# artiom-matvei/RLAO

Measured on NVIDIA B200. Metric: closed-loop AO env-steps/sec (batched envs), higher is better.
Workload: dtype f32

## Files before the change

### include/aoenv.h

```cpp
#ifndef AOENV_H_
#define AOENV_H_

#include <stdint.h>

#ifdef __cplusplus
extern "C" {
#endif

#define AOENV_MAX_LAYERS 8
#define AOENV_ABI_VERSION 1

int aoenv_abi_version(void);
const char* aoenv_last_error(void);
uint64_t aoenv_launch_count(void);
int aoenv_set_pdl(int enabled);


int aoenv_atm_gather(const float* win, int B, int M, int pitch, int64_t env_stride, int sx, int sy,
                     const int32_t* inner_rc, int nI, int nO, const float* xi,
                     uint64_t seed, uint64_t stream_id, float* zx, int ldz, void* zx_planes, int parts, void* stream);

int aoenv_atm_ring(float* win, int B, int M, int pitch, int64_t env_stride, int64_t win_offset, int nO, const float* X,
                   int ldx, uint64_t* ext, int32_t* flag, int force_rescan, void* stream);

int aoenv_atm_gather_multi(const void* const* wins, const int32_t* sx, const int32_t* sy, const uint64_t* seeds,
                           const uint64_t* stream_ids, int G, int B, int M, int pitch, int64_t env_stride,
                           const int32_t* inner_rc, int nI, int nO, const float* xi, float* zx, int ldz,
                           void* zx_planes, int parts, void* stream);
int aoenv_atm_ring_multi(void* const* wins, const int64_t* win_offsets, void* const* exts, int G, int B, int M,
                         int pitch, int64_t env_stride, int nO, const float* X, int ldx, int32_t* flag,
                         int force_rescan, void* stream);

int aoenv_atm_gather_envs(const void* const* wins, const uint64_t* seeds, const uint64_t* stream_ids, int G,
                          const int32_t* env_idx, int k, int M, int pitch, int64_t env_stride, const int32_t* inner_rc,
                          int nI, int nO, float* zx, int ldz, void* zx_planes, int parts, void* stream);
int aoenv_atm_ring_envs(void* const* wins, const int64_t* win_offsets, void* const* exts, int G, const int32_t* env_idx,
                        int k, int B, int M, int pitch, int64_t env_stride, int nO, const float* X, int ldx, int32_t* flag,
                        void* stream);

int aoenv_atm_compact(const float* src_win, float* dst_win, int B, int M, int pitch, int64_t env_stride, uint64_t* ext,
                      int64_t pos_delta, void* stream);

int aoenv_vk_screens(uint64_t seed, uint32_t screen0, int S, int N, const float* amp, const float* inject, const void* wa_planes,
                     const void* wb_planes, int Kp, int parts, const float* sh_ex, const float* sh_ey, const float* h_amp,
                     const float* h_mx, const float* h_my, void* work_planes, float* work_a, int lda, float* work_b, int ldb,
                     float* dst, int pitch, int64_t env_stride, void* stream);

int aoenv_vk_screens_envs(uint64_t seed, uint32_t screen0, const int32_t* env_idx, int S, int N, const float* amp,
                          const void* wa_planes, const void* wb_planes, int Kp, int parts, const float* sh_ex,
                          const float* sh_ey, const float* h_amp, const float* h_mx, const float* h_my, void* work_planes,
                          float* work_a, int lda, float* work_b, int ldb, float* dst, int pitch, int64_t env_stride,
                          void* stream);

int aoenv_atm_phase(const float* const* h_canvas, const uint64_t* const* h_ext, const int32_t* h_org, int nLayer, int B,
                    int R, int M, int Mc, int pitch, int fp_off, const int32_t* h_row_off, const int32_t* h_col_off,
                    const float* h_wrow, const float* h_wcol, const float* h_weight, float opd_scale, float* opd_out,
                    void* stream);
int aoenv_atm_phase_envs(const float* const* h_canvas, const uint64_t* const* h_ext, const int32_t* h_org, int nLayer,
                         int B, int R, int M, int Mc, int pitch, int fp_off, const int32_t* h_row_off,
                         const int32_t* h_col_off, const float* h_wrow, const float* h_wcol, const float* h_weight,
                         float opd_scale, const int32_t* env_idx, int k, float* opd_out, void* stream);

typedef struct {
  double ratio[2];
  double buff[2];
  double vX, vY;
  uint64_t events;
  uint64_t philox_seed;
  int32_t not_done_once;
  int32_t cur;
  int32_t org[2];
} aoenv_layer_state_t;

typedef struct {
  int32_t nLayer, B, R, M, Mc, pitch, S, nI, nO, ldz, ldx, group_max, parts, fp_off, warp_kernel, use_tc;
  int64_t env_stride;
  uint64_t env_offset;
  double sampling_time, ps_loop;
  float opd_scale, reserved;
  float weight[AOENV_MAX_LAYERS];
  void* maps[AOENV_MAX_LAYERS][2];
  void* ext[AOENV_MAX_LAYERS];
  const void* inner_rc;
  void* zx;
  void* zx_planes;
  void* X;
  void* flag;
  const void* w_f32;
  aoenv_layer_state_t layer[AOENV_MAX_LAYERS];
} aoenv_atm_state_t;

int aoenv_atm_update(aoenv_atm_state_t* state, const void* w_planes, float* opd_out, void* stream);

#define AOENV_SKINNY_MAX_ROWS 8
int aoenv_gemm_tn(const float* X, int ldx, const float* W, int ldw, float* D, int ldd,
                  int M, int N, int K, float alpha, void* stream);

int aoenv_split_bf16(const float* src, int lds, int rows, int K, int parts, void* dst, int ldk, void* stream);
int aoenv_gemm_tn_tc(const void* Xs, const void* Ws, int ldk, int parts, float* D, int ldd, int MX, int NW, int K,
                     float alpha, void* stream);

int aoenv_dm_surface_separable(const float* coefs, int ldc, const int32_t* act_pos, int nA, int nAct, const float* gx,
                               const float* gy, const int32_t* band_x, const int32_t* band_y, const float* wx,
                               const int32_t* j0x, const float* wyp, const int32_t* i0y, int W, int B, int R, float* opd,
                               void* stream);

typedef struct {
  int32_t photon_noise;
  int32_t sensor_emccd;
  int32_t has_fwc;
  int32_t bits;
  float qe;
  float dark_electrons;
  float fwc;
  float gain;
  float readout_noise;
  uint32_t reserved;
  uint64_t seed;
  uint64_t frame_counter;
} aoenv_detector_t;

int aoenv_detector_integrate(float* frame, int B, int rows, int cols, const aoenv_detector_t* det, void* stream);

int aoenv_shwfs_camera(float* frame, const uint8_t* valid, int B, int nS, int n, const aoenv_detector_t* det, int shared_max,
                       int32_t* envmax, void* stream);

int aoenv_set_wfs6_variant(int variant);

int aoenv_shwfs_frame(const float* opd_a, const float* opd_b, const float* pupil, const float* amp,
                      const uint8_t* valid, int B, int nS, int n, float phase_scale,
                      const aoenv_detector_t* det, int shared_max,
                      float* frame, int32_t* envmax, double* stats, void* stream);

int aoenv_shwfs_slopes(const float* frame, const int32_t* envmax, int shared_max, const int32_t* valid_idx,
                       int nV, const float* ref_xy, float inv_units, float threshold_cog, int B, int nS, int n,
                       float* slopes, int lds, void* slope_planes, int parts, void* stream);

typedef struct {
  const float* rows;
  const float* wlr;
  const int32_t* ilr;
  int32_t nActP;
  int32_t WL;
  int32_t t_rows;
  int32_t reserved;
} aoenv_dm_sep_t;

int aoenv_shwfs_fused(const float* opd_a, const float* opd_b, const aoenv_dm_sep_t* dm, const uint8_t* pupil8, float amp0,
                      const int32_t* h_row_start, const int32_t* order, const int32_t* nlit, const int32_t* slot_of, int B,
                      int nS, int n, int cluster, int groups, float phase_scale, const float* ref_xy, int nV, float inv_units,
                      float threshold_cog, float* frame, float* slopes, int lds, void* slope_planes, int parts,
                      int32_t* envmax, double* stats, void* stream);
int aoenv_shwfs_frame_dm(const float* opd_a, const float* opd_b, const aoenv_dm_sep_t* dm, const int32_t* order,
                         const float* pupil, const float* amp, const uint8_t* valid, int B, int nS, int n, float phase_scale,
                         const aoenv_detector_t* det, int shared_max, float* frame, int32_t* envmax, double* stats,
                         void* stream);
int aoenv_shwfs_fused_smem(int nS, int n, int rows_max, int groups, int t_rows, int WL);
int aoenv_dm_rows(const float* coefs, int ldc, const int32_t* act_pos, int nA, int nAct, int nActP, const float* wx,
                  const int32_t* j0x, int W, int B, int R, float* rows, void* stream);

typedef struct {
  int32_t B, nS, n, nV, lds, nA, nAct, nAct2, ldc, ldr, W, rec_parts, use_tc, geometric;
  float phase_scale, inv_units, threshold_cog, leak;
  double n_pupil;
  const void *pupil, *amp, *valid, *order, *valid_idx, *ref_xy;
  void *frame, *envmax, *stats, *slopes, *slope_planes;
  aoenv_dm_sep_t dm;
  const void *rec_planes, *rec_f32;
  void* rec;
  const void* act_idx;
  void* dm_prev;
  const void *act_pos, *wx, *j0x;
} aoenv_sh_step_t;

int aoenv_sh_step(const aoenv_sh_step_t* c, int parts, const float* opd_a, const float* dm_rows_cur, const aoenv_detector_t* det,
                  const float* action, float* coefs_next, float* dm_rows_next, float* obs, float* reward, float* strehl,
                  float* total, float* residual, void* stream);

int aoenv_shwfs_measure_f64(const float* opd, const float* pupil, const float* amp, const uint8_t* valid,
                            const int32_t* valid_idx, int nV, const double* ref_xy, double inv_units, double threshold_cog,
                            int F, int nS, int n, double phase_scale, int shared_max, double* frame, uint64_t* envmax,
                            double* slopes, int lds, void* stream);

int aoenv_shwfs_geometric(const float* opd_a, const float* opd_b, const aoenv_dm_sep_t* dm, const float* pupil,
                          const float* flux, const int32_t* valid_idx, int nV, int B, int nS, int n, float phase_scale,
                          float inv_units, float* slopes, int lds, void* slope_planes, int parts, double* stats, void* stream);

int aoenv_shwfs_geometric_f64(const float* opd, const float* flux, const int32_t* valid_idx, int nV, int F, int nS, int n,
                              double phase_scale, double inv_units, double* slopes, int lds, void* stream);

int aoenv_pyramid_supported(int N);
int aoenv_pyramid_frames(const float* opd_a, const float* opd_b, const float* pupil, const float* amp, const float* lin,
                         const float* mod, const float* mask_s, int B, int R, int N, int nTheta, int bin, float phase_scale,
                         float* work_x1, float* work_yt, float* intensity, float* frame, void* stream);


int aoenv_command_update(const float* action, const int32_t* act_idx, int B, int nA, int nAct2, float leak,
                         float* coefs, float* dm_prev, int ldc, void* stream);

int aoenv_observe(const float* rec, int ldr, const int32_t* act_idx, int B, int nA, int nAct2,
                  const double* stats, double n_pupil, float phase_scale,
                  float* obs, float* reward, float* strehl, float* total, float* residual, void* stream);

int aoenv_normal_fill(uint64_t seed, uint64_t counter, int rows, int cols, int ld, float sigma, float* out, void* planes,
                      int parts, void* stream);
int aoenv_vec_to_img(const float* vec, int ldv, const int32_t* act_idx, int B, int nA, int nAct2, float scale, float* img,
                     void* stream);

int aoenv_psf_peak(const float* opd_a, const float* opd_b, const float* pupil, const float* amp,
                   const void* w1_planes, const float* g2, int B, int R, int N, int os, int win, float phase_scale,
                   void* field_planes, int ldk, float* scratch, float* psf_win, float* psf_max, void* stream);

int aoenv_psf_image(const float* opd_a, const float* opd_b, const float* pupil, const float* amp, const void* w_planes, int B,
                    int R, int N, int os, int win, float phase_scale, void* field_planes, int ldk, float* work_t, void* planes_u,
                    float* work_f, float* psf, float* psf_max, void* stream);

#ifdef __cplusplus
}
#endif
#endif
```

### rlao_b200/OOPAOEnv/OOPAOEnvRazor.py

```python
import contextlib
import ctypes
import importlib
import math
import os
import types

import numpy as np
import torch

from .. import _lib, gemm
from ..Atmosphere import Atmosphere
from ..DeformableMirror import DeformableMirror, DMSurfaceRef
from ..MisRegistration import MisRegistration
from ..ShackHartmann import ShackHartmann
from ..Source import Source
from ..Telescope import Telescope
from ..Zernike import Zernike
from ..calibration.CalibrationVault import CalibrationVault
from ..calibration.InteractionMatrix import InteractionMatrix
from ..tools import linalg


_NVTX = os.environ.get("AOENV_NVTX", "0") not in ("", "0")

# ... 121 lines not shown
        else:
            M2C = torch.eye(self.dm.nValidAct, dtype=torch.float64, device=self.device)
        calib_zonal = InteractionMatrix(ngs=self.source, atm=self.atm, tel=self.tel, dm=self.dm, wfs=self.wfs,
                                        M2C=torch.eye(self.dm.nValidAct, dtype=torch.float64, device=self.device),
                                        stroke=1e-9, nMeasurements=param.get("nMeasurements", 25), noise="off")
        self.calib_zonal = calib_zonal
        calib = CalibrationVault(calib_zonal.D @ M2C)
        self.tel.resetOPD()
        self.dm.coefs = 0
        self._dm_prev = torch.zeros((self.n_envs, self.dm._Kp), dtype=torch.float32, device=self.device)
        self._coefs_buf = torch.zeros((2, self.n_envs, self.dm._Kp), dtype=torch.float32, device=self.device)
        self._coefs_slot = 0
        self.source * self.tel * self.dm * self.wfs
        self.tel + self.atm
        self.calib_CL = calib
        self.M2C_CL = M2C
        nLoop = param.get("nLoop", None)
        self.SR = []
        self._nLoop = nLoop
        self.total = torch.zeros((nLoop, self.n_envs), dtype=torch.float32, device=self.device) if nLoop else None
        self.residual = torch.zeros((nLoop, self.n_envs), dtype=torch.float32, device=self.device) if nLoop else None
        cam.photonNoise = param.get("cam_photonNoise", True)
        cam.readoutNoise = param.get("cam_readoutNoise", 14 if wfs_type == "shackhartmann" else 0)
        self.set_reconstructor(M2C @ calib.M)
        self.F = M2C @ linalg.pinv(M2C)
        nA_, Kp_ = self.dm.nValidAct, self.dm._Kp
        self._F32 = torch.zeros((nA_, Kp_), dtype=torch.float32, device=self.device)
        self._F32[:, :nA_] = self.F.to(torch.float32)
        self._F_op = gemm.Operator(self._F32, parts=2)
        self.dm.free_float64()
        B, nA = self.n_envs, self.dm.nValidAct
        self._act_idx = torch.as_tensor((self.xvalid * nAct + self.yvalid).astype(np.int32), device=self.device)
        self._rec = torch.zeros((B, (nA + 3) // 4 * 4), dtype=torch.float32, device=self.device)
        self._obs = torch.zeros((B, nAct, nAct), dtype=torch.float32, device=self.device)
        self._reward = torch.zeros((B,), dtype=torch.float32, device=self.device)
        self._strehl = torch.zeros((B,), dtype=torch.float32, device=self.device)
        self._total_now = torch.zeros((B,), dtype=torch.float32, device=self.device)
        self._residual_now = torch.zeros((B,), dtype=torch.float32, device=self.device)
        self._phase_scale = 2 * math.pi / self.source.wavelength
        self._noise_seed = (seed * 7919 + 5) & 0xFFFFFFFFFFFFFFFF
        self._noise_calls = 0
        self._noise_z = torch.zeros((B, self.dm._Kp), dtype=torch.float32, device=self.device)
        self._noise_planes = torch.zeros((2, B, self.dm._Kp), dtype=torch.bfloat16, device=self.device)
        self._noise_vec = torch.zeros((B, (nA + 3) // 4 * 4), dtype=torch.float32, device=self.device)

    def set_reconstructor(self, R):
        self.reconstructor = torch.as_tensor(R, dtype=torch.float64, device=self.device)
        nA, nSig = self.reconstructor.shape
        self._Rm = torch.zeros((nA, self.wfs._lds), dtype=torch.float32, device=self.device)
        self._Rm[:, :nSig] = self.reconstructor.to(torch.float32)
        self._Rm_op = gemm.Operator(self._Rm, parts=2)

    @property
    def dm_prev(self):
        d = self._dm_prev[:, :self.dm.nValidAct]
        return d[0] if self.n_envs == 1 else d

    @dm_prev.setter
    def dm_prev(self, val):
        t = torch.as_tensor(val, dtype=torch.float32, device=self.device)
        self._dm_prev.zero_()
        self._dm_prev[:, :self.dm.nValidAct] = t

    def _sq(self, t):
        return t[0] if self.n_envs == 1 else t

    def _observe(self, with_stats):
        lib, st, B, nA = _lib.load(), _lib.stream_ptr(self.device), self.n_envs, self.dm.nValidAct
        sig = self.wfs._signal
        gemm.gemm_tn(sig, self._Rm_op, self._rec, B, nA,
                     x_planes=self.wfs._signal_planes if gemm.uses_tensor_cores(B) else None)
        _lib.check(lib.aoenv_observe(_lib.ptr(self._rec), self._rec.stride(0), _lib.ptr(self._act_idx), B, nA,
                                     self.nActuator ** 2, _lib.ptr(self.wfs._stats) if with_stats else None,
                                     float(self.tel.pixelArea), self._phase_scale, _lib.ptr(self._obs), _lib.ptr(self._reward),
                                     _lib.ptr(self._strehl), _lib.ptr(self._total_now), _lib.ptr(self._residual_now), st),
                   "observe")

    def _action_tensor(self, action):
        a = torch.as_tensor(action, dtype=torch.float32, device=self.device)
        nAct = self.nActuator
        if a.ndim == 2:
            a = a.unsqueeze(0).expand(self.n_envs, -1, -1)
        return a.reshape(self.n_envs, nAct * nAct).contiguous()

    def reset_soft(self):
        self.action_buffer = []
        self._observe(False)
        return self._sq(self._obs).clone()

    def reset(self):
        raise NotImplementedError("reset() rebuilds the whole simulation in the reference (set_params without arguments, "
                                  "OOPAOEnvRazor.py:66-71, which raises there too); use set_params(...) then reset_soft()")

    def reset_envs(self, env_ids, seed):
        atm, dm = self.atm, self.dm
        atm._check_partial_reset()
        idx = atm.env_index(env_ids)
        if idx.numel() == 0:
            return idx
        if dm._coefs_matrix is not None or dm._multi is not None:
            raise NotImplementedError("reset_envs needs per-environment commands (the mirror holds a calibration command matrix)")
        atm._reset_listed(idx, seed)
        rows = idx.long()
        slot = dm._slot
        self._dm_prev[rows] = 0
        for c in {id(t): t for t in (dm._coefs, dm._coefs_of[slot]) if t is not None}.values():
            c[rows] = 0
        if dm._rows is not None and dm._rows_valid[slot]:
            dm._rows[slot][rows] = 0
        if dm._valid[slot]:
            dm._opd[slot][rows] = 0
        return idx

    def reset_soft_wfs(self):
        self.action_buffer = []
        return self.wfs.cam.frame.clone()

    def _native_cfg(self):
        wfs, dm, tel = self.wfs, self.dm, self.tel
        if (not self.native_step or _NVTX or self.psf_reward is not None or type(wfs) is not ShackHartmann or wfs.use_fused
                or not wfs.inline_dm or not dm.lazy_surface or self.atm.user_defined_opd or dm._multi is not None
                or dm._coefs_matrix is not None):
            return None
        src = tel.src
        if wfs._flux_version != getattr(src, "_flux_version", 0) or wfs.current_nPhoton != src.nPhoton:
            return None
        key = (wfs._flux_version, wfs.is_geometric, id(wfs._amp), id(wfs._ref_xy), wfs.slopes_units, wfs.threshold_cog, float(self.leak),
               id(self._Rm_op), id(dm._sep), src.wavelength, id(self._coefs_buf))
        if self._native_key == key:
            return self._native
        self._native_key, self._native = key, None
        tables = dm.fused_tables()
        win = wfs._dm_windows(tables) if tables is not None else None
        if win is None or 2 * math.pi / src.wavelength != self._phase_scale:
            return None
        tc = gemm.uses_tensor_cores(self.n_envs)
        dm._rows_of(dm._slot)
        c = _lib.ShStepStruct()
        c.B, c.nS, c.n, c.nV, c.lds = self.n_envs, wfs.nSubap, wfs.n_pix_subap, wfs.nValidSubaperture, wfs._signal.stride(0)
        c.nA, c.nAct, c.nAct2 = dm.nValidAct, dm.nAct, self.nActuator ** 2
        c.ldc, c.ldr, c.W, c.rec_parts, c.use_tc = self._coefs_buf.stride(1), self._rec.stride(0), tables["W"], self._Rm_op.parts, int(tc)
        c.geometric = int(wfs.is_geometric)
        c.phase_scale, c.inv_units, c.threshold_cog, c.leak = self._phase_scale, 1.0 / wfs.slopes_units, wfs.threshold_cog, self.leak
        c.n_pupil = float(tel.pixelArea)
        keep = [tel._pupil_f, wfs._amp, wfs._valid_u8, wfs._lit_first, wfs._valid_idx, wfs._ref_xy, wfs._frame, wfs._envmax,
                wfs._stats, wfs._signal, wfs._signal_planes, win, self._Rm, self._Rm_op, self._rec, self._act_idx, self._dm_prev,
                tables]
        c.pupil, c.amp, c.valid, c.order = tel._pupil_f.data_ptr(), wfs._amp.data_ptr(), wfs._valid_u8.data_ptr(), wfs._lit_first.data_ptr()
        c.valid_idx, c.ref_xy, c.envmax = wfs._valid_idx.data_ptr(), wfs._ref_xy.data_ptr(), wfs._envmax.data_ptr()
        if wfs.is_geometric:
            c.amp, c.frame = wfs._flux.data_ptr(), None
            keep.append(wfs._flux)
        else:
            c.frame = wfs._frame.data_ptr()
        c.stats, c.slopes, c.slope_planes = wfs._stats.data_ptr(), wfs._signal.data_ptr(), wfs._signal_planes.data_ptr()
        c.dm.wlr, c.dm.ilr, c.dm.nActP, c.dm.WL = win[2].data_ptr(), win[1].data_ptr(), dm._rows.shape[2], win[0]
        c.rec_planes = self._Rm_op.planes().data_ptr() if tc else None
        c.rec_f32, c.rec, c.act_idx, c.dm_prev = self._Rm.data_ptr(), self._rec.data_ptr(), self._act_idx.data_ptr(), self._dm_prev.data_ptr()
        c.act_pos, c.wx, c.j0x = tables["act_pos"].data_ptr(), tables["wx"].data_ptr(), tables["j0x"].data_ptr()
        self._native = (c, keep)
        return self._native

    def _step_native(self, i, action, native, action_ready=None, after_observe=None):
        c = native[0]
        dm, wfs, atm, B, dev = self.dm, self.wfs, self.atm, self.n_envs, self.device
        slot = dm._slot
        atm.update()
        self.tel._set_lazy(atm._opd, DMSurfaceRef(dm, slot))
        det = None if wfs.is_geometric else wfs.cam.as_struct(self.env_offset)
        nAct = self.nActuator
        obs = torch.empty((B, nAct, nAct), dtype=torch.float32, device=dev)
        reward = torch.empty((B,), dtype=torch.float32, device=dev)
        strehl = torch.empty((B,), dtype=torch.float32, device=dev)
        coefs = self._coefs_buf[self._coefs_slot]
        args = [atm._opd.data_ptr(), dm._rows[slot].data_ptr(), ctypes.byref(det) if det is not None else None, None,
                coefs.data_ptr(), dm._rows[slot ^ 1].data_ptr(), obs.data_ptr(), reward.data_ptr(), strehl.data_ptr(),
                self._total_now.data_ptr(), self._residual_now.data_ptr(), _lib.stream_ptr(dev)]
        step, cref = _lib.load().aoenv_sh_step, ctypes.byref(c)
        if atm.can_prefetch() or after_observe is not None or action_ready is not None:
            early = atm.sm_partition is not None or (self.prefetch_early and after_observe is None and action_ready is None)
            if early:
                atm.prefetch()
            _lib.check(step(cref, 1, *args), "sh_step")
            if not early:
                atm.prefetch()
            _lib.check(step(cref, 2, *args), "sh_step")
            if after_observe is not None:
                after_observe(self._sq(obs), self._sq(reward), self._sq(strehl))
            if action_ready is not None:
                torch.cuda.current_stream(dev).wait_event(action_ready)
            args[3] = self._action_tensor(action).data_ptr()
            _lib.check(step(cref, 4, *args), "sh_step")
        else:
            act = self._action_tensor(action)
            args[3] = act.data_ptr()
            _lib.check(step(cref, 7, *args), "sh_step")
        self._coefs_slot ^= 1
        dm._coefs, dm._multi, dm._coefs_matrix, dm._slot = coefs, None, None, slot ^ 1
        dm._coefs_of[slot ^ 1], dm._rows_valid[slot ^ 1], dm._valid[slot ^ 1] = coefs, True, False
        if not wfs.is_geometric:
            wfs.cam.frame = wfs._frame[0] if B == 1 else wfs._frame
        wfs._signal_is_multi = False
        self._obs, self._reward, self._strehl = obs, reward, strehl
        if self.total is not None and i is not None and 0 <= i < self._nLoop:
            self.total[i] = self._total_now
            self.residual[i] = self._residual_now
        s = self._sq(strehl)
        self.SR.append(s)
        self.wfsSignal = wfs.signal
        return self._sq(obs), self._sq(reward), s, False, {"strehl": s}

    def step(self, i, action):
        native = self._native_cfg()
        if native is not None and self.dm._rows_valid[self.dm._slot]:
            return self._step_native(i, action, native)
        obs, reward, strehl, done, info = self._measure_frame(i)
        self._apply_command(action)
        strehl = strehl.clone()
        self.SR[-1] = strehl
        return obs.clone(), reward.clone(), strehl, done, {"strehl": strehl}

    def _step_views(self, i, action, action_ready=None, after_observe=None):
        native = self._native_cfg()
        if native is not None and self.dm._rows_valid[self.dm._slot]:
            return self._step_native(i, action, native, action_ready, after_observe)
        out = self._measure_frame(i, after_observe)
        self._apply_command(action, action_ready)
        return out

    def _measure_frame(self, i, after_observe=None, atmosphere_done=False):
        if not atmosphere_done:
            with _range("aoenv.atmosphere"):
                self.atm.update()
        else:
            self.atm._join_prefetch(consume=True)
        dm_surface = self.dm.surface_ref()
        self.tel._set_lazy(self.atm._opd, dm_surface)
        with _range("aoenv.wfs"):
            self.wfs._measure_terms(self.atm._opd, dm_surface, self.env_offset)
        if not atmosphere_done:
            with _range("aoenv.atmosphere_next"):
                self.atm.prefetch()
        with _range("aoenv.reconstruct"):
            self._observe(True)
        if self.total is not None and i is not None and 0 <= i < self._nLoop:
            self.total[i] = self._total_now
            self.residual[i] = self._residual_now
        strehl = self._sq(self._strehl)
        if self.psf_reward is not None:
            strehl = self.psf_strehl(*self.psf_reward)
        if after_observe is not None:
            after_observe(self._sq(self._obs), self._sq(self._reward), strehl)
        self.SR.append(strehl if self.psf_reward is not None else strehl.clone())
        self.wfsSignal = self.wfs.signal
        return self._sq(self._obs), self._sq(self._reward), strehl, False, {"strehl": strehl}

    def _apply_command(self, action, action_ready=None):
        lib, st, B = _lib.load(), _lib.stream_ptr(self.device), self.n_envs
        if action_ready is not None:
            torch.cuda.current_stream(self.device).wait_event(action_ready)
        action = self._action_tensor(action)
        coefs = self._coefs_buf[self._coefs_slot]
        self._coefs_slot ^= 1
        with _range("aoenv.command"):
            _lib.check(lib.aoenv_command_update(_lib.ptr(action), _lib.ptr(self._act_idx), B, self.dm.nValidAct,
                                                self.nActuator ** 2, ctypes.c_float(self.leak), _lib.ptr(coefs), _lib.ptr(self._dm_prev),
                                                coefs.stride(0), st), "command_update")
            self.dm._set_coefs_batch(coefs)

    def state_dict(self):
        atm = self.atm
        nxt = None
        if atm._prefetched:
            atm._wait_prefetch()
            nxt = atm._opd_next.detach().cpu().clone()
        layers = []
        for i, ly in enumerate(atm._layers):
            layers.append(dict(map=ly.mapShift.detach().cpu().clone(), buff=ly.buff.copy(), ratio=ly.ratio.copy(),
                               notDoneOnce=ly.notDoneOnce, events=ly.events, philox_seed=getattr(ly, "philox_seed", 0),
                               ext=None))
        return dict(version=1, n_envs=self.n_envs, rng=atm.rng, layers=layers, atm_opd=atm._opd.detach().cpu().clone(),
                    atm_opd_next=nxt,
                    coefs=self.dm._coefs.detach().cpu().clone(), dm_prev=self._dm_prev.detach().cpu().clone(),
                    cam_frame_counter=self.wfs.cam.frame_counter, noise_calls=self._noise_calls,
                    SR=[s.detach().cpu().clone() for s in self.SR],
                    total=None if self.total is None else self.total.detach().cpu().clone(),
                    residual=None if self.residual is None else self.residual.detach().cpu().clone())

    def load_state_dict(self, st):
        if st.get("version") != 1 or st["n_envs"] != self.n_envs or st["rng"] != self.atm.rng:
            raise ValueError("state_dict of another environment (n_envs / rng / version differ)")
        if self.atm.rng != "philox":
            raise NotImplementedError("host MT19937 streams (rng='reference') are not checkpointed; use rng='philox'")
        atm, dev = self.atm, self.device
        atm._join_prefetch(consume=False)
        for i, (ly, s_) in enumerate(zip(atm._layers, st["layers"])):
            atm._cur[i] = 0
            atm._org[i] = atm._fresh_origin(i)
            oy, ox = atm._org[i]
            m = s_["map"].to(dev)
            atm._maps[i, 0, :, oy:oy + atm._M, ox:ox + atm._M] = m if m.ndim == 3 else m.unsqueeze(0)
            ly.buff, ly.ratio, ly.notDoneOnce = s_["buff"].copy(), s_["ratio"].copy(), s_["notDoneOnce"]
            ly.events, ly.philox_seed = s_["events"], s_["philox_seed"]
            atm._rescan_extrema(i)
        atm._opd.copy_(st["atm_opd"].to(dev))
        if st.get("atm_opd_next") is not None:
            if atm._opd_next is None:
# ... 145 lines not shown
```

### rlao_b200/ShackHartmann.py

```python
import ctypes as C
import math
import os

import numpy as np
import torch

from . import _lib, gemm
from .DeformableMirror import DMSurfaceRef
from .Detector import Detector

_SUPPORTED_N = (4, 6, 8)


class ShackHartmann:
    def __init__(self, nSubap, telescope, lightRatio, threshold_cog=0.01, is_geometric=False, binning_factor=1,
                 padding_extension_factor=1, threshold_convolution=0.05, shannon_sampling=False, unit_P2V=False):
        self.tag = "shackHartmann"
        self.telescope = telescope
        if telescope.src is None:
            raise AttributeError("The telescope was not coupled to any source object! Make sure to couple it with an src object using src*tel")
        if binning_factor != 1 or padding_extension_factor > 2:
            raise NotImplementedError("binning_factor != 1 / extended field of view are out of scope")
        if getattr(telescope.src, "type", "NGS") == "LGS":
            raise NotImplementedError("LGS spot elongation is out of scope")
        self.device = telescope.device
        self.n_envs = telescope.n_envs
        self._is_geometric = bool(is_geometric)
        self.nSubap = int(nSubap)
        self._lightRatio = lightRatio
        self.binning_factor = 1
        self.zero_padding = 2
        self.padding_extension_factor = padding_extension_factor
        self.threshold_convolution = threshold_convolution
        self.threshold_cog = threshold_cog
        self.shannon_sampling = shannon_sampling
        self.unit_P2V = unit_P2V
        R = telescope.resolution
        if R % self.nSubap != 0:
            raise ValueError("telescope.resolution must be a multiple of nSubap")
        self.n_pix_subap = R // self.nSubap
        if self.n_pix_subap not in _SUPPORTED_N:
            raise NotImplementedError(f"{self.n_pix_subap} pixels per subaperture: compiled sizes are {_SUPPORTED_N}")
        self.n_pix_subap_init = self.n_pix_subap
        self.n_pix_lenslet_init = self.n_pix_subap * self.zero_padding
        self.n_pix_lenslet = self.n_pix_lenslet_init
        self.is_extended = False
        self.is_LGS = False
        self.cam = Detector(round(self.nSubap * self.n_pix_subap))
        self.cam.photonNoise = 0
        self.cam.readoutNoise = 0
        src = telescope.src
        self.fov_lenslet_arcsec = (self.n_pix_subap * 206265 * self.binning_factor / self.padding_extension_factor
                                   * src.wavelength / (telescope.D / self.nSubap)) / (1 + self.shannon_sampling)
        self.fov_pixel_arcsec = self.fov_lenslet_arcsec / self.n_pix_subap
        self.fov_pixel_binned_arcsec = self.fov_lenslet_arcsec / self.n_pix_subap_init
        self.get_camera_frame_multi = False
        self.env_offset = 0
        self.use_fused = os.environ.get("AOENV_WFS", "kernels") == "fused" and not self._is_geometric
        self.keep_frame = False
        self._fused_plans = {}
        self.inline_dm = os.environ.get("AOENV_WFS_INLINE_DM", "1") != "0"
        self._dm_window_cache = {}
        self._last_inputs = None
        ii, jj = np.meshgrid(np.arange(self.nSubap), np.arange(self.nSubap), indexing="ij")
        self.index_x, self.index_y = ii.reshape(-1), jj.reshape(-1)
        self.initialize_flux()
        self._select_valid()
        B = self.n_envs
        self._frame = None if self._is_geometric else torch.zeros((B, R, R), dtype=torch.float32, device=self.device)
        self._envmax = torch.zeros((B,), dtype=torch.int32, device=self.device)
        self._stats = torch.zeros((B, 4), dtype=torch.float64, device=self.device)
        self._signal = torch.zeros((B, self._lds), dtype=torch.float32, device=self.device)
        self._signal_planes = torch.zeros((2, B, self._lds), dtype=torch.bfloat16, device=self.device)
        self._signal_is_multi = False
        self.initialize_wfs()

    def initialize_flux(self, input_flux_map=None):
        src, nS, n = self.telescope.src, self.nSubap, self.n_pix_subap
        flux = np.asarray(src.fluxMap if input_flux_map is None else input_flux_map.T, dtype=np.float64)
        self.photon_per_subaperture = flux.reshape(nS, n, nS, n).sum(axis=(1, 3)).reshape(-1)
        self.photon_per_subaperture_2D = self.photon_per_subaperture.reshape(nS, nS)
        self._amp = torch.as_tensor(np.sqrt(flux), dtype=torch.float32, device=self.device).contiguous()
        if self._is_geometric:
            self._flux = torch.as_tensor(flux, dtype=torch.float32, device=self.device).contiguous()
        self.current_nPhoton = src.nPhoton
        self._flux_version = getattr(src, "_flux_version", 0)
        pup = np.asarray(self.telescope.pupil)
        inside = pup > 0
        vals = flux[inside]
        self._uniform_flux = bool(inside.any() and np.all((pup == 0) | (pup == 1)) and np.all(flux[~inside] == 0)
                                  and np.all(vals == vals[0]))
        self._amp0 = float(np.sqrt(vals[0])) if self._uniform_flux else 0.0
        self._pupil8 = torch.as_tensor(inside.astype(np.uint8), device=self.device).contiguous()

    def _select_valid(self):
        nS = self.nSubap
        pps = self.photon_per_subaperture
        self.valid_subapertures = (pps >= self._lightRatio * pps.max()).reshape(nS, nS)
        self.valid_subapertures_1D = self.valid_subapertures.reshape(-1)
        self.validLenslets_x, self.validLenslets_y = np.where(self.valid_subapertures)
        self.valid_slopes_maps = np.concatenate((self.valid_subapertures, self.valid_subapertures))
        self.nValidSubaperture = int(self.valid_subapertures.sum())
        self.nSignal = 2 * self.nValidSubaperture
        self._lds = (self.nSignal + 15) // 16 * 16
        dev = self.device
        self._valid_u8 = torch.as_tensor(self.valid_subapertures_1D.astype(np.uint8), device=dev).contiguous()
        self._valid_idx = torch.as_tensor(np.nonzero(self.valid_subapertures_1D)[0].astype(np.int32), device=dev).contiguous()
        slot = np.full(nS * nS, -1, dtype=np.int32)
        slot[np.nonzero(self.valid_subapertures_1D)[0]] = np.arange(self.nValidSubaperture, dtype=np.int32)
        self._slot_of = torch.as_tensor(slot, device=dev).contiguous()
        v1 = np.asarray(self.valid_subapertures_1D).astype(bool).reshape(-1)
        self._lit_first = torch.as_tensor(np.concatenate([np.nonzero(v1)[0], np.nonzero(~v1)[0]]).astype(np.int32),
                                          device=dev).contiguous()
        self._fused_plans = {}

    @property
    def lightRatio(self):
        return self._lightRatio

    @lightRatio.setter
    def lightRatio(self, val):
        self._lightRatio = val
        self._select_valid()
        self._signal = torch.zeros((self.n_envs, self._lds), dtype=torch.float32, device=self.device)
        self._signal_planes = torch.zeros((2, self.n_envs, self._lds), dtype=torch.bfloat16, device=self.device)
        self.initialize_wfs()

    @property
    def is_geometric(self):
        return self._is_geometric

    @is_geometric.setter
    def is_geometric(self, val):
        if bool(val) != self._is_geometric:
            raise NotImplementedError("the calibration (reference, slope units) belongs to the sensor mode: build a new "
                                      "ShackHartmann(is_geometric=...) instead of switching it")

    def _dm_windows_host(self, dm_tables):
        nS, n = self.nSubap, self.n_pix_subap
        R = nS * n
        by, gy = dm_tables["by_host"], dm_tables["gy_host"]
        lo = by[:, 0].reshape(nS, n).min(axis=1)
        hi = by[:, 1].reshape(nS, n).max(axis=1)
        need = int((hi - lo + 1).max())
        WL = 14 if need <= 14 else (18 if need <= 18 else 0)
        if WL == 0:
            return 0, None, None
        half = (WL + 1) // 2
        hp = (half + 3) // 4 * 4
        wl = np.zeros((R, 2 * hp), dtype=np.float32)
        for y in range(R):
            i0 = lo[y // n]
            for i in range(by[y, 0], by[y, 1] + 1):
                t = i - i0
                wl[y, (t // half) * hp + t % half] = gy[i, y]
        return WL, lo.astype(np.int32), wl

    def _dm_windows(self, dm_tables):
        key = id(dm_tables)
        hit = self._dm_window_cache.get(key)
        if hit is None:
            WL, ilr, wlr = self._dm_windows_host(dm_tables)
            hit = (WL, None, None) if WL == 0 else (
                WL, torch.as_tensor(ilr, dtype=torch.int32, device=self.device).contiguous(),
                torch.as_tensor(wlr, dtype=torch.float32, device=self.device).contiguous())
            self._dm_window_cache[key] = (hit, dm_tables)
        else:
            hit = hit[0]
        return hit if hit[0] != 0 else None

    def _fused_plan(self, dm_tables):
        key = id(dm_tables) if dm_tables is not None else 0
        plan = self._fused_plans.get(key)
        if plan is not None:
            return plan
        lib, nS, n, dev = _lib.load(), self.nSubap, self.n_pix_subap, self.device
        R = nS * n
        groups = int(os.environ.get("AOENV_WFS_GROUPS", "4"))
        valid = self.valid_subapertures
        lit_row = valid.sum(axis=1).astype(np.float64)
        WL, ilr, wlr = 0, None, None
        if dm_tables is not None:
            WL, ilr, wlr = self._dm_windows_host(dm_tables)
            if WL == 0:
                raise NotImplementedError("DM influence bands are too wide for the fused kernel")

        def t_rows_for(rs):
            if ilr is None:
                return 0
            return int(max(ilr[rs[k + 1] - 1] + WL - ilr[rs[k]] for k in range(len(rs) - 1)))

        Cmax = min(16, nS)
        cost = 0.26 * nS + lit_row
        pre = np.concatenate([[0.0], np.cumsum(cost)])
        seg = pre[None, :] - pre[:, None]
        best = np.full((Cmax + 1, nS + 1), np.inf)
        arg = np.zeros((Cmax + 1, nS + 1), dtype=np.int64)
        best[0, 0] = 0.0
        for c in range(1, Cmax + 1):
            for e in range(c, nS + 1):
                v = np.maximum(best[c - 1, c - 1:e], seg[c - 1:e, e])
                k = int(np.argmin(v))
                best[c, e], arg[c, e] = v[k], c - 1 + k

        def partition(C_):
            rs, e = [nS], nS
            for c in range(C_, 0, -1):
                e = int(arg[c, e])
                rs.append(e)
            return rs[::-1]

        def smem_for(rs):
            rows_max = max(rs[k + 1] - rs[k] for k in range(len(rs) - 1))
            return lib.aoenv_shwfs_fused_smem(nS, n, rows_max, groups, t_rows_for(rs), WL)
        forced = os.environ.get("AOENV_WFS_CLUSTER")
        limit = 227 * 1024
        cands = {c: partition(c) for c in range(1, Cmax + 1)}
        if forced:
            cluster = int(forced)
        else:
            fit8 = [c for c in cands if c <= 8 and 0 < smem_for(cands[c]) <= limit]
            good = [c for c in fit8 if nS * nS // c >= 96]
            if good:
# ... 268 lines not shown
```

### rlao_b200/_lib.py

```python
import ctypes as C
import os

import torch

_HERE = os.path.dirname(os.path.abspath(__file__))
LIB_PATH = os.path.join(_HERE, "libaoenv_b200.so")


class AOEnvLibraryError(RuntimeError):
    pass


class DetectorStruct(C.Structure):
    _fields_ = [
        ("photon_noise", C.c_int32), ("sensor_emccd", C.c_int32), ("has_fwc", C.c_int32), ("bits", C.c_int32),
        ("qe", C.c_float), ("dark_electrons", C.c_float), ("fwc", C.c_float), ("gain", C.c_float),
        ("readout_noise", C.c_float), ("reserved", C.c_uint32), ("seed", C.c_uint64), ("frame_counter", C.c_uint64),
    ]


class DmSepStruct(C.Structure):
    _fields_ = [
        ("rows", C.c_void_p), ("wlr", C.c_void_p), ("ilr", C.c_void_p),
        ("nActP", C.c_int32), ("WL", C.c_int32), ("t_rows", C.c_int32), ("reserved", C.c_int32),
    ]


MAX_LAYERS = 8


class LayerState(C.Structure):
    _fields_ = [
        ("ratio", C.c_double * 2), ("buff", C.c_double * 2), ("vX", C.c_double), ("vY", C.c_double),
        ("events", C.c_uint64), ("philox_seed", C.c_uint64),
        ("not_done_once", C.c_int32), ("cur", C.c_int32), ("org", C.c_int32 * 2),
    ]


class ShStepStruct(C.Structure):
    _fields_ = [(k, C.c_int32) for k in ("B", "nS", "n", "nV", "lds", "nA", "nAct", "nAct2", "ldc", "ldr", "W", "rec_parts",
                                         "use_tc", "geometric")] + [
        ("phase_scale", C.c_float), ("inv_units", C.c_float), ("threshold_cog", C.c_float), ("leak", C.c_float),
        ("n_pupil", C.c_double)] + [(k, C.c_void_p) for k in ("pupil", "amp", "valid", "order", "valid_idx", "ref_xy", "frame",
                                                              "envmax", "stats", "slopes", "slope_planes")] + [
        ("dm", DmSepStruct)] + [(k, C.c_void_p) for k in ("rec_planes", "rec_f32", "rec", "act_idx", "dm_prev", "act_pos",
                                                           "wx", "j0x")]


class AtmState(C.Structure):
    _fields_ = [(k, C.c_int32) for k in ("nLayer", "B", "R", "M", "Mc", "pitch", "S", "nI", "nO", "ldz", "ldx", "group_max",
                                         "parts", "fp_off", "warp_kernel", "use_tc")] + [
        ("env_stride", C.c_int64), ("env_offset", C.c_uint64), ("sampling_time", C.c_double), ("ps_loop", C.c_double),
        ("opd_scale", C.c_float), ("reserved", C.c_float), ("weight", C.c_float * MAX_LAYERS),
        ("maps", (C.c_void_p * 2) * MAX_LAYERS), ("ext", C.c_void_p * MAX_LAYERS), ("inner_rc", C.c_void_p),
        ("zx", C.c_void_p), ("zx_planes", C.c_void_p), ("X", C.c_void_p), ("flag", C.c_void_p), ("w_f32", C.c_void_p),
        ("layer", LayerState * MAX_LAYERS),
    ]

_vp, _i, _f, _u64, _d, _i64 = C.c_void_p, C.c_int, C.c_float, C.c_uint64, C.c_double, C.c_int64

PROTOTYPES = {
    "aoenv_atm_gather": [_vp, _i, _i, _i, _i64, _i, _i, _vp, _i, _i, _vp, _u64, _u64, _vp, _i, _vp, _i, _vp],
    "aoenv_atm_ring": [_vp, _i, _i, _i, _i64, _i64, _i, _vp, _i, _vp, _vp, _i, _vp],
    "aoenv_atm_gather_multi": [_vp, _vp, _vp, _vp, _vp, _i, _i, _i, _i, _i64, _vp, _i, _i, _vp, _vp, _i, _vp, _i, _vp],
    "aoenv_atm_ring_multi": [_vp, _vp, _vp, _i, _i, _i, _i, _i64, _i, _vp, _i, _vp, _i, _vp],
    "aoenv_atm_gather_envs": [_vp, _vp, _vp, _i, _vp, _i, _i, _i, _i64, _vp, _i, _i, _vp, _i, _vp, _i, _vp],
    "aoenv_atm_ring_envs": [_vp, _vp, _vp, _i, _vp, _i, _i, _i, _i, _i64, _i, _vp, _i, _vp, _vp],
    "aoenv_atm_compact": [_vp, _vp, _i, _i, _i, _i64, _vp, _i64, _vp],
    "aoenv_vk_screens": [_u64, C.c_uint32, _i, _i, _vp, _vp, _vp, _vp, _i, _i, _vp, _vp, _vp, _vp, _vp, _vp, _vp, _i, _vp, _i,
                         _vp, _i, _i64, _vp],
    "aoenv_vk_screens_envs": [_u64, C.c_uint32, _vp, _i, _i, _vp, _vp, _vp, _i, _i, _vp, _vp, _vp, _vp, _vp, _vp, _vp, _i, _vp,
                              _i, _vp, _i, _i64, _vp],
    "aoenv_atm_update": [_vp, _vp, _vp, _vp],
    "aoenv_sh_step": [_vp, _i] + [_vp] * 12,
    "aoenv_atm_phase": [_vp, _vp, _vp, _i, _i, _i, _i, _i, _i, _i, _vp, _vp, _vp, _vp, _vp, _f, _vp, _vp],
    "aoenv_atm_phase_envs": [_vp, _vp, _vp, _i, _i, _i, _i, _i, _i, _i, _vp, _vp, _vp, _vp, _vp, _f, _vp, _i, _vp, _vp],
    "aoenv_gemm_tn": [_vp, _i, _vp, _i, _vp, _i, _i, _i, _i, _f, _vp],
    "aoenv_split_bf16": [_vp, _i, _i, _i, _i, _vp, _i, _vp],
    "aoenv_gemm_tn_tc": [_vp, _vp, _i, _i, _vp, _i, _i, _i, _i, _f, _vp],
    "aoenv_dm_surface_separable": [_vp, _i, _vp, _i, _i, _vp, _vp, _vp, _vp, _vp, _vp, _vp, _vp, _i, _i, _i, _vp, _vp],
    "aoenv_set_wfs6_variant": [_i],
    "aoenv_detector_integrate": [_vp, _i, _i, _i, _vp, _vp],
    "aoenv_shwfs_camera": [_vp, _vp, _i, _i, _i, _vp, _i, _vp, _vp],
    "aoenv_shwfs_frame": [_vp, _vp, _vp, _vp, _vp, _i, _i, _i, _f, _vp, _i, _vp, _vp, _vp, _vp],
    "aoenv_shwfs_frame_dm": [_vp, _vp, _vp, _vp, _vp, _vp, _vp, _i, _i, _i, _f, _vp, _i, _vp, _vp, _vp, _vp],
    "aoenv_shwfs_slopes": [_vp, _vp, _i, _vp, _i, _vp, _f, _f, _i, _i, _i, _vp, _i, _vp, _i, _vp],
    "aoenv_shwfs_fused": [_vp, _vp, _vp, _vp, _f, _vp, _vp, _vp, _vp, _i, _i, _i, _i, _i, _f, _vp, _i, _f, _f, _vp, _vp, _i, _vp, _i,
                          _vp, _vp, _vp],
    "aoenv_shwfs_fused_smem": [_i, _i, _i, _i, _i, _i],
    "aoenv_dm_rows": [_vp, _i, _vp, _i, _i, _i, _vp, _vp, _i, _i, _i, _vp, _vp],
    "aoenv_shwfs_geometric": [_vp, _vp, _vp, _vp, _vp, _vp, _i, _i, _i, _i, _f, _f, _vp, _i, _vp, _i, _vp, _vp],
    "aoenv_shwfs_geometric_f64": [_vp, _vp, _vp, _i, _i, _i, _i, _d, _d, _vp, _i, _vp],
    "aoenv_shwfs_measure_f64": [_vp, _vp, _vp, _vp, _vp, _i, _vp, _d, _d, _i, _i, _i, _d, _i, _vp, _vp, _vp, _i, _vp],
    "aoenv_normal_fill": [_u64, _u64, _i, _i, _i, _f, _vp, _vp, _i, _vp],
    "aoenv_vec_to_img": [_vp, _i, _vp, _i, _i, _i, _f, _vp, _vp],
    "aoenv_pyramid_supported": [_i],
    "aoenv_pyramid_frames": [_vp, _vp, _vp, _vp, _vp, _vp, _vp, _i, _i, _i, _i, _i, _f, _vp, _vp, _vp, _vp, _vp],
    "aoenv_command_update": [_vp, _vp, _i, _i, _i, _f, _vp, _vp, _i, _vp],
    "aoenv_observe": [_vp, _i, _vp, _i, _i, _i, _vp, _d, _f, _vp, _vp, _vp, _vp, _vp, _vp],
    "aoenv_psf_image": [_vp, _vp, _vp, _vp, _vp, _i, _i, _i, _i, _i, _f, _vp, _i, _vp, _vp, _vp, _vp, _vp, _vp],
    "aoenv_psf_peak": [_vp, _vp, _vp, _vp, _vp, _vp, _i, _i, _i, _i, _i, _f, _vp, _i, _vp, _vp, _vp, _vp],
}

_lib = None


def load():
    global _lib
    if _lib is not None:
        return _lib
    if not os.path.exists(LIB_PATH):
        raise AOEnvLibraryError(
            f"{LIB_PATH} not found: the CUDA extension has not been built. Build it with "
            "`bash rlao_b200/csrc/build.sh` (needs nvcc with sm_100a support). rlao_b200 has no CPU fallback.")
    lib = C.CDLL(LIB_PATH)
    lib.aoenv_abi_version.restype = C.c_int
    lib.aoenv_last_error.restype = C.c_char_p
    lib.aoenv_launch_count.restype = C.c_uint64
    lib.aoenv_set_pdl.argtypes, lib.aoenv_set_pdl.restype = [C.c_int], C.c_int
    for name, args in PROTOTYPES.items():
        fn = getattr(lib, name)
        fn.argtypes = args
        fn.restype = C.c_int
    _lib = lib
    return lib


def check(rc, what=""):
    if rc != 0:
        raise RuntimeError(f"libaoenv_b200 {what} failed ({rc}): {load().aoenv_last_error().decode()}")


def ptr(t):
    return None if t is None else t.data_ptr()


_raw_stream = getattr(torch._C, "_cuda_getCurrentRawStream", None)


def stream_ptr(device=None):
    if _raw_stream is not None:
        if device is None:
            idx = torch.cuda.current_device()
        else:
            idx = device.index if isinstance(device, torch.device) else torch.device(device).index
            if idx is None:
                idx = torch.cuda.current_device()
        return _raw_stream(idx)
    return torch.cuda.current_stream(device).cuda_stream


def launch_count():
    return int(load().aoenv_launch_count())


def require_cuda(device):
    if not torch.cuda.is_available():
        raise AOEnvLibraryError("rlao_b200 needs a CUDA device (B200, sm_100a); there is no CPU fallback")
    dev = torch.device(device if device is not None else "cuda:0")
    if dev.type != "cuda":
        raise AOEnvLibraryError(f"rlao_b200 objects live on CUDA devices, got {dev}")
    return dev
```

### rlao_b200/csrc/common.cuh

```cuda
#pragma once
#include <cuda_bf16.h>
#include <cuda_runtime.h>
#include <stdint.h>
#include <stdio.h>
#include <atomic>

#include "../../include/aoenv.h"

namespace aoenv {

extern thread_local char g_err[512];
extern std::atomic<uint64_t> g_launches;

int fail(int code, const char* fmt, ...);

#define AOENV_CHECK_ARG(cond, ...)                         \
  do {                                                     \
    if (!(cond)) return ::aoenv::fail(-2, __VA_ARGS__);    \
  } while (0)

#define AOENV_LAUNCH_CHECK(name)                                                        \
  do {                                                                                  \
    ::aoenv::g_launches.fetch_add(1, std::memory_order_relaxed);                        \
    cudaError_t e__ = cudaGetLastError();                                               \
    if (e__ != cudaSuccess) return ::aoenv::fail(-3, "%s: %s", name, cudaGetErrorString(e__)); \
  } while (0)

constexpr int kNumSMs = 148;

extern int g_pdl;
__device__ __forceinline__ void pdl_enter() {
  asm volatile("griddepcontrol.launch_dependents;" ::: "memory");
  asm volatile("griddepcontrol.wait;" ::: "memory");
}
__device__ __forceinline__ void pdl_trigger() { asm volatile("griddepcontrol.launch_dependents;" ::: "memory"); }
__device__ __forceinline__ void pdl_wait() { asm volatile("griddepcontrol.wait;" ::: "memory"); }

struct PdlLaunch {
  cudaLaunchConfig_t cfg;
  cudaLaunchAttribute attr[1];
  PdlLaunch(dim3 grid, dim3 block, size_t smem, cudaStream_t stream) {
    cfg = cudaLaunchConfig_t{};
    cfg.gridDim = grid;
    cfg.blockDim = block;
    cfg.dynamicSmemBytes = smem;
    cfg.stream = stream;
    attr[0].id = cudaLaunchAttributeProgrammaticStreamSerialization;
    attr[0].val.programmaticStreamSerializationAllowed = g_pdl;
    cfg.attrs = attr;
    cfg.numAttrs = 1;
  }
};
#define AOENV_LAUNCH(kernel, grid, block, smem, stream, ...)                  \
  do {                                                                        \
    ::aoenv::PdlLaunch l__(grid, block, smem, stream);                        \
    cudaLaunchKernelEx(&l__.cfg, kernel, __VA_ARGS__);                        \
  } while (0)

__device__ __forceinline__ int32_t float_to_ordered(float f) {
  int32_t i = __float_as_int(f);
  return i >= 0 ? i : i ^ 0x7fffffff;
}
__device__ __forceinline__ float ordered_to_float(int32_t i) {
  return __int_as_float(i >= 0 ? i : i ^ 0x7fffffff);
}

__device__ __forceinline__ float warp_sum(float v) {
#pragma unroll
  for (int o = 16; o > 0; o >>= 1) v += __shfl_xor_sync(0xffffffffu, v, o);
  return v;
}
__device__ __forceinline__ double warp_sum(double v) {
#pragma unroll
  for (int o = 16; o > 0; o >>= 1) v += __shfl_xor_sync(0xffffffffu, v, o);
  return v;
}
__device__ __forceinline__ float warp_max(float v) {
#pragma unroll
  for (int o = 16; o > 0; o >>= 1) v = fmaxf(v, __shfl_xor_sync(0xffffffffu, v, o));
  return v;
}
__device__ __forceinline__ float warp_min(float v) {
#pragma unroll
  for (int o = 16; o > 0; o >>= 1) v = fminf(v, __shfl_xor_sync(0xffffffffu, v, o));
  return v;
}

__device__ __forceinline__ float2 fma2(float2 a, float2 b, float2 c) {
  unsigned long long d;
  asm("fma.rn.f32x2 %0, %1, %2, %3;" : "=l"(d) : "l"(*reinterpret_cast<unsigned long long*>(&a)),
      "l"(*reinterpret_cast<unsigned long long*>(&b)), "l"(*reinterpret_cast<unsigned long long*>(&c)));
  return *reinterpret_cast<float2*>(&d);
}
__device__ __forceinline__ float2 add2(float2 a, float2 b) {
  unsigned long long d;
  asm("add.rn.f32x2 %0, %1, %2;" : "=l"(d) : "l"(*reinterpret_cast<unsigned long long*>(&a)),
      "l"(*reinterpret_cast<unsigned long long*>(&b)));
  return *reinterpret_cast<float2*>(&d);
}
__device__ __forceinline__ float2 sub2(float2 a, float2 b) {
  unsigned long long d;
  asm("sub.rn.f32x2 %0, %1, %2;" : "=l"(d) : "l"(*reinterpret_cast<unsigned long long*>(&a)),
      "l"(*reinterpret_cast<unsigned long long*>(&b)));
  return *reinterpret_cast<float2*>(&d);
}
__device__ __forceinline__ float2 mul2(float2 a, float2 b) {
  unsigned long long d;
  asm("mul.rn.f32x2 %0, %1, %2;" : "=l"(d) : "l"(*reinterpret_cast<unsigned long long*>(&a)),
      "l"(*reinterpret_cast<unsigned long long*>(&b)));
  return *reinterpret_cast<float2*>(&d);
}
__device__ __forceinline__ float2 dup2(float s) { return make_float2(s, s); }

struct Philox {
  uint32_t key[2];
  __device__ __forceinline__ Philox(uint64_t seed) {
    key[0] = (uint32_t)seed;
    key[1] = (uint32_t)(seed >> 32);
  }
  __device__ __forceinline__ uint4 operator()(uint32_t c0, uint32_t c1, uint32_t c2, uint32_t c3) const {
    uint32_t k0 = key[0], k1 = key[1];
#pragma unroll
    for (int r = 0; r < 10; ++r) {
      const uint32_t hi0 = __umulhi(0xD2511F53u, c0), lo0 = 0xD2511F53u * c0;
      const uint32_t hi1 = __umulhi(0xCD9E8D57u, c2), lo1 = 0xCD9E8D57u * c2;
      const uint32_t n0 = hi1 ^ c1 ^ k0, n2 = hi0 ^ c3 ^ k1;
      c0 = n0; c1 = lo1; c2 = n2; c3 = lo0;
      k0 += 0x9E3779B9u; k1 += 0xBB67AE85u;
    }
    return make_uint4(c0, c1, c2, c3);
  }
};

__device__ __forceinline__ float u32_to_unit(uint32_t x) { return ((float)(x >> 8) + 1.0f) * (1.0f / 16777216.0f); }

__device__ __forceinline__ float2 box_muller(uint32_t a, uint32_t b) {
  const float u1 = u32_to_unit(a);
  const float u2 = u32_to_unit(b);
  const float r = sqrtf(-2.0f * logf(u1));
  float s, c;
  sincospif(2.0f * u2, &s, &c);
  return make_float2(r * c, r * s);
}

__device__ __forceinline__ void store_bf16_planes(__nv_bfloat16* __restrict__ planes, size_t plane_stride, size_t idx,
                                                  int parts, float x) {
  for (int p = 0; p < parts; ++p) {
    const __nv_bfloat16 h = __float2bfloat16_rn(x);
    planes[(size_t)p * plane_stride + idx] = h;
    x -= __bfloat162float(h);
  }
}

}
```

### rlao_b200/csrc/ctrl.cu

```cuda
#include "common.cuh"

namespace aoenv {

__global__ void __launch_bounds__(256)
command_update_kernel(const float* __restrict__ action, const int32_t* __restrict__ act_idx, int nA, int nAct2,
                      float leak, float* __restrict__ coefs, float* __restrict__ dm_prev, int ldc) {
  pdl_enter();
  const int b = blockIdx.y;
  const int a = blockIdx.x * blockDim.x + threadIdx.x;
  if (a >= nA) return;
  const float act = __ldg(&action[(size_t)b * nAct2 + __ldg(&act_idx[a])]) * 1e-6f;
  const float c = dm_prev[(size_t)b * ldc + a] * leak + act;
  coefs[(size_t)b * ldc + a] = c;
  dm_prev[(size_t)b * ldc + a] = c;
}

__global__ void __launch_bounds__(256)
observe_kernel(const float* __restrict__ rec, int ldr, const int32_t* __restrict__ act_idx, int nA, int nAct2,
               const double* __restrict__ stats, double n_pupil, float phase_scale, float* __restrict__ obs,
               float* __restrict__ reward, float* __restrict__ strehl, float* __restrict__ total,
               float* __restrict__ residual) {
  pdl_enter();
  const int b = blockIdx.x;
  float* __restrict__ o = obs + (size_t)b * nAct2;
  for (int i = threadIdx.x; i < nAct2; i += blockDim.x) o[i] = 0.f;
  __syncthreads();
  float ss = 0.f;
  for (int a = threadIdx.x; a < nA; a += blockDim.x) {
    const float v = -__ldg(&rec[(size_t)b * ldr + a]) * 1e6f;
    o[__ldg(&act_idx[a])] = v;
    ss = fmaf(v, v, ss);
  }
  ss = warp_sum(ss);
  __shared__ float sh[8];
  if ((threadIdx.x & 31) == 0) sh[threadIdx.x >> 5] = ss;
  __syncthreads();
  if (threadIdx.x == 0) {
    float t = 0.f;
    for (int w = 0; w < (int)(blockDim.x >> 5); ++w) t += sh[w];
    reward[b] = -sqrtf(t);
    if (stats != nullptr) {
      const double* s = stats + (size_t)b * 4;
      const double ma = s[0] / n_pupil, va = fmax(s[1] / n_pupil - ma * ma, 0.0);
      const double mt = s[2] / n_pupil, vt = fmax(s[3] / n_pupil - mt * mt, 0.0);
      total[b] = (float)(sqrt(va) * 1e9);
      residual[b] = (float)(sqrt(vt) * 1e9);
      strehl[b] = (float)exp(-vt * (double)phase_scale * (double)phase_scale);
    }
  }
}

__global__ void __launch_bounds__(256)
normal_fill_kernel(unsigned long long seed, unsigned long long counter, int rows, int cols, int ld, float sigma,
                   float* __restrict__ out, __nv_bfloat16* __restrict__ planes, int parts) {
  const int r = blockIdx.y;
  const int q = blockIdx.x * blockDim.x + threadIdx.x;
  if (4 * q >= ld) return;
  Philox rng(seed);
  const uint4 w = rng((uint32_t)q, (uint32_t)r, (uint32_t)counter, (uint32_t)(counter >> 32));
  const float2 n0 = box_muller(w.x, w.y), n1 = box_muller(w.z, w.w);
  const float v[4] = {n0.x, n0.y, n1.x, n1.y};
#pragma unroll
  for (int k = 0; k < 4; ++k) {
    const int c = 4 * q + k;
    if (c >= ld) break;
    const float x = c < cols ? v[k] * sigma : 0.f;
    out[(size_t)r * ld + c] = x;
    if (planes != nullptr) store_bf16_planes(planes, (size_t)rows * ld, (size_t)r * ld + c, parts, x);
  }
}

__global__ void __launch_bounds__(256)
vec_to_img_kernel(const float* __restrict__ vec, int ldv, const int32_t* __restrict__ act_idx, int nA, int nAct2, float scale,
                  float* __restrict__ img) {
  const int b = blockIdx.x;
  float* __restrict__ o = img + (size_t)b * nAct2;
  for (int i = threadIdx.x; i < nAct2; i += blockDim.x) o[i] = 0.f;
  __syncthreads();
  for (int a = threadIdx.x; a < nA; a += blockDim.x) o[__ldg(&act_idx[a])] = __ldg(&vec[(size_t)b * ldv + a]) * scale;
}

}

using namespace aoenv;

extern "C" {

int aoenv_command_update(const float* action, const int32_t* act_idx, int B, int nA, int nAct2, float leak,
                         float* coefs, float* dm_prev, int ldc, void* stream) {
  AOENV_CHECK_ARG(B > 0 && B <= 65535 && nA > 0 && ldc >= nA, "command_update: bad shape");
  dim3 grid((nA + 255) / 256, B);
  AOENV_LAUNCH(command_update_kernel, grid, 256, 0, (cudaStream_t)stream, action, act_idx, nA, nAct2, leak, coefs, dm_prev, ldc);
  AOENV_LAUNCH_CHECK("command_update");
  return 0;
}

int aoenv_normal_fill(uint64_t seed, uint64_t counter, int rows, int cols, int ld, float sigma, float* out, void* planes,
                      int parts, void* stream) {
  AOENV_CHECK_ARG(rows > 0 && rows <= 65535 && cols > 0 && ld >= cols, "normal_fill: bad shape rows=%d cols=%d ld=%d", rows, cols, ld);
  AOENV_CHECK_ARG(planes == nullptr || parts == 2 || parts == 3, "normal_fill: parts must be 2 or 3");
  dim3 grid(((ld + 3) / 4 + 255) / 256, rows);
  normal_fill_kernel<<<grid, 256, 0, (cudaStream_t)stream>>>(seed, counter, rows, cols, ld, sigma, out, (__nv_bfloat16*)planes, parts);
  AOENV_LAUNCH_CHECK("normal_fill");
  return 0;
}

int aoenv_vec_to_img(const float* vec, int ldv, const int32_t* act_idx, int B, int nA, int nAct2, float scale, float* img,
                     void* stream) {
  AOENV_CHECK_ARG(B > 0 && nA > 0 && ldv >= nA && nAct2 >= nA, "vec_to_img: bad shape");
  vec_to_img_kernel<<<B, 256, 0, (cudaStream_t)stream>>>(vec, ldv, act_idx, nA, nAct2, scale, img);
  AOENV_LAUNCH_CHECK("vec_to_img");
  return 0;
}

int aoenv_observe(const float* rec, int ldr, const int32_t* act_idx, int B, int nA, int nAct2, const double* stats,
                  double n_pupil, float phase_scale, float* obs, float* reward, float* strehl, float* total,
                  float* residual, void* stream) {
  AOENV_CHECK_ARG(B > 0 && nA > 0 && ldr >= nA, "observe: bad shape");
  AOENV_LAUNCH(observe_kernel, dim3(B), 256, 0, (cudaStream_t)stream, rec, ldr, act_idx, nA, nAct2, stats, n_pupil, phase_scale, obs,
                                                      reward, strehl, total, residual);
  AOENV_LAUNCH_CHECK("observe");
  return 0;
}

}
```

### rlao_b200/csrc/step.cu

```cuda
#include <math.h>
#include <string.h>

#include "common.cuh"

using namespace aoenv;

namespace {

struct Step { int sx, sy; };

inline double sign_of(double v) { return v > 0 ? 1.0 : (v < 0 ? -1.0 : 0.0); }

int plan_layer(const aoenv_atm_state_t& st, aoenv_layer_state_t& ly, Step* steps, int max_steps) {
  int count = 0;
  if (ly.vX == 0.0 && ly.vY == 0.0) return 0;
  if (ly.not_done_once) {
    ly.not_done_once = 0;
    ly.ratio[0] = ly.vX * st.sampling_time / st.ps_loop;
    ly.ratio[1] = ly.vY * st.sampling_time / st.ps_loop;
    ly.buff[0] = ly.buff[1] = 0.0;
  }
  double a[2] = {fabs(ly.ratio[0]), fabs(ly.ratio[1])};
  long n[2];
  for (int k = 0; k < 2; ++k) n[k] = isinf(a[k]) ? 0 : (long)a[k];
  const double sg[2] = {sign_of(ly.ratio[0]), sign_of(ly.ratio[1])};
  const long nmin = n[0] < n[1] ? n[0] : n[1], nmax = n[0] < n[1] ? n[1] : n[0];
  for (long r = 0; r < nmin && count < max_steps; ++r) steps[count++] = {(int)sg[0], (int)sg[1]};
  for (long r = 0; r < nmax - nmin && count < max_steps; ++r)
    steps[count++] = {n[0] == nmin ? 0 : (int)sg[0], n[1] == nmin ? 0 : (int)sg[1]};
  if (nmax > max_steps) return -1;
  for (int k = 0; k < 2; ++k) ly.buff[k] += fmod(fabs(ly.ratio[k]), 1.0) * sg[k];
  if (fabs(ly.buff[0]) >= 1.0 || fabs(ly.buff[1]) >= 1.0) {
    if (count >= max_steps) return -1;
    steps[count++] = {fabs(ly.buff[0]) < 1.0 ? 0 : (int)sign_of(ly.buff[0]), fabs(ly.buff[1]) < 1.0 ? 0 : (int)sign_of(ly.buff[1])};
  }
  for (int k = 0; k < 2; ++k) ly.buff[k] = fmod(fabs(ly.buff[k]), 1.0) * sign_of(ly.buff[k]);
  return count;
}

inline int pick_origin(double v, int S, int align) {
  const int o = v > 0 ? S : (v < 0 ? 0 : S / 2);
  return o / align * align;
}

inline float* window(const aoenv_atm_state_t& st, int i, int buf, int oy, int ox) {
  return (float*)st.maps[i][buf] + ((size_t)oy * st.pitch + ox);
}

void tap_weights(double buff, int kernel, int* off, float* w) {
  const double f = floor(-buff), frac = -buff - f;
  *off = (int)f - 1;
  double x, v[4];
  if (kernel == 0) {
    x = (frac + 1.0) / 3.0;
    v[0] = 1.0 + x * (-5.5 + x * (9.0 + x * -4.5));
    v[1] = x * (9.0 + x * (-22.5 + x * 13.5));
    v[2] = x * (-4.5 + x * (18.0 + x * -13.5));
    v[3] = x * (1.0 + x * (-4.5 + x * 4.5));
  } else {
    x = frac;
    v[0] = 0.5 * x * (-1.0 + x * (2.0 - x));
    v[1] = 1.0 + 0.5 * x * x * (-5.0 + 3.0 * x);
    v[2] = 0.5 * x * (1.0 + x * (4.0 - 3.0 * x));
    v[3] = 0.5 * x * x * (x - 1.0);
  }
  for (int k = 0; k < 4; ++k) w[k] = (float)v[k];
}

int extrude_group(aoenv_atm_state_t& st, const int* layers, const Step* steps, int G, const void* w_planes, void* stream) {
  const void* wins[AOENV_MAX_LAYERS];
  int32_t sxs[AOENV_MAX_LAYERS], sys_[AOENV_MAX_LAYERS];
  uint64_t seeds[AOENV_MAX_LAYERS], ids[AOENV_MAX_LAYERS];
  const int S = st.S;
  for (int g = 0; g < G; ++g) {
    const int i = layers[g];
    aoenv_layer_state_t& ly = st.layer[i];
    const int sx = steps[g].sx, sy = steps[g].sy;
    if (!(0 <= ly.org[0] - sy && ly.org[0] - sy <= S && 0 <= ly.org[1] - sx && ly.org[1] - sx <= S)) {
      const int foy = pick_origin(ly.vY, S, 1), fox = pick_origin(ly.vX, S, 4);
      int rc = aoenv_atm_compact(window(st, i, ly.cur, ly.org[0], ly.org[1]), window(st, i, 1 - ly.cur, foy, fox), st.B, st.M,
                                 st.pitch, st.env_stride, (uint64_t*)st.ext[i],
                                 (int64_t)(foy - ly.org[0]) * st.pitch + (fox - ly.org[1]), stream);
      if (rc) return rc;
      ly.cur = 1 - ly.cur;
      ly.org[0] = foy;
      ly.org[1] = fox;
      if (!(0 <= foy - sy && foy - sy <= S && 0 <= fox - sx && fox - sx <= S))
        return fail(-2, "atm_update: canvas slack too small for this wind direction change");
    }
    wins[g] = window(st, i, ly.cur, ly.org[0], ly.org[1]);
    sxs[g] = sx;
    sys_[g] = sy;
    seeds[g] = ly.philox_seed;
    ids[g] = ((ly.events << 8) | (uint64_t)i) + (st.env_offset << 40);
    ly.events += 1;
  }
  const bool tc = st.use_tc && G * st.B > AOENV_SKINNY_MAX_ROWS;
  int rc = aoenv_atm_gather_multi(wins, sxs, sys_, seeds, ids, G, st.B, st.M, st.pitch, st.env_stride, (const int32_t*)st.inner_rc,
                                  st.nI, st.nO, nullptr, tc ? nullptr : (float*)st.zx, st.ldz, tc ? st.zx_planes : nullptr,
                                  st.parts, stream);
  if (rc) return rc;
  if (tc)
    rc = aoenv_gemm_tn_tc(st.zx_planes, w_planes, st.ldz, st.parts, (float*)st.X, st.ldx, G * st.B, st.nO, st.ldz, 1.0f, stream);
  else
    rc = aoenv_gemm_tn((const float*)st.zx, st.ldz, (const float*)st.w_f32, st.ldz, (float*)st.X, st.ldx, G * st.B, st.nO, st.ldz,
                       1.0f, stream);
  if (rc) return rc;
  void* wins2[AOENV_MAX_LAYERS];
  int64_t offs[AOENV_MAX_LAYERS];
  void* exts[AOENV_MAX_LAYERS];
  for (int g = 0; g < G; ++g) {
    aoenv_layer_state_t& ly = st.layer[layers[g]];
    ly.org[0] -= steps[g].sy;
    ly.org[1] -= steps[g].sx;
    wins2[g] = window(st, layers[g], ly.cur, ly.org[0], ly.org[1]);
    offs[g] = (int64_t)ly.org[0] * st.pitch + ly.org[1];
    exts[g] = st.ext[layers[g]];
  }
  return aoenv_atm_ring_multi(wins2, offs, exts, G, st.B, st.M, st.pitch, st.env_stride, st.nO, (const float*)st.X, st.ldx,
                              (int32_t*)st.flag, 0, stream);
}

}

extern "C" {

int aoenv_atm_update(aoenv_atm_state_t* state, const void* w_planes, float* opd_out, void* stream) {
  AOENV_CHECK_ARG(state != nullptr && opd_out != nullptr, "atm_update: null state / output");
  aoenv_atm_state_t& st = *state;
  const int L = st.nLayer;
  AOENV_CHECK_ARG(L >= 1 && L <= AOENV_MAX_LAYERS && st.group_max >= 1, "atm_update: %d layers", L);
  AOENV_CHECK_ARG(!st.use_tc || w_planes != nullptr, "atm_update: the operator planes are missing");
  constexpr int kMaxSteps = 64;
  static thread_local Step plans[AOENV_MAX_LAYERS][kMaxSteps];
  int count[AOENV_MAX_LAYERS], rounds = 0;
  for (int i = 0; i < L; ++i) {
    count[i] = plan_layer(st, st.layer[i], plans[i], kMaxSteps);
    if (count[i] < 0) return fail(-2, "atm_update: more than %d add_row steps in one frame (layer %d)", kMaxSteps, i);
    if (count[i] > rounds) rounds = count[i];
  }
  for (int r = 0; r < rounds; ++r) {
    int layers[AOENV_MAX_LAYERS], G = 0;
    Step steps[AOENV_MAX_LAYERS];
    for (int i = 0; i < L; ++i)
      if (count[i] > r) {
        layers[G] = i;
        steps[G++] = plans[i][r];
      }
    for (int k = 0; k < G; k += st.group_max) {
      const int g = G - k < st.group_max ? G - k : st.group_max;
      const int rc = extrude_group(st, layers + k, steps + k, g, w_planes, stream);
      if (rc) return rc;
    }
  }
  const float* canv[AOENV_MAX_LAYERS];
  const uint64_t* exts[AOENV_MAX_LAYERS];
  int32_t org[2 * AOENV_MAX_LAYERS], roff[AOENV_MAX_LAYERS], coff[AOENV_MAX_LAYERS];
  float wr[4 * AOENV_MAX_LAYERS], wc[4 * AOENV_MAX_LAYERS];
  for (int i = 0; i < L; ++i) {
    const aoenv_layer_state_t& ly = st.layer[i];
    canv[i] = (const float*)st.maps[i][ly.cur];
    exts[i] = (const uint64_t*)st.ext[i];
    org[2 * i] = ly.org[0];
    org[2 * i + 1] = ly.org[1];
    tap_weights(ly.buff[0], st.warp_kernel, &coff[i], &wc[4 * i]);
    tap_weights(ly.buff[1], st.warp_kernel, &roff[i], &wr[4 * i]);
  }
  return aoenv_atm_phase(canv, exts, org, L, st.B, st.R, st.M, st.Mc, st.pitch, st.fp_off, roff, coff, wr, wc, st.weight,
                         st.opd_scale, opd_out, stream);
}

}

extern "C" int aoenv_sh_step(const aoenv_sh_step_t* c, int parts, const float* opd_a, const float* dm_rows_cur,
                             const aoenv_detector_t* det, const float* action, float* coefs_next, float* dm_rows_next,
                             float* obs, float* reward, float* strehl, float* total, float* residual, void* stream) {
  AOENV_CHECK_ARG(c != nullptr && parts >= 1 && parts <= 7, "sh_step: bad arguments");
  AOENV_CHECK_ARG(!(parts & 1) || (opd_a != nullptr && dm_rows_cur != nullptr), "sh_step: null wavefront argument");
  AOENV_CHECK_ARG(!(parts & 2) || (obs != nullptr && reward != nullptr && strehl != nullptr), "sh_step: null output argument");
  AOENV_CHECK_ARG(!(parts & 4) || (action != nullptr && coefs_next != nullptr && dm_rows_next != nullptr), "sh_step: null command argument");
  const bool tc = c->use_tc && c->B > AOENV_SKINNY_MAX_ROWS;
  int rc = 0;
  if ((parts & 1) && c->geometric) {
    aoenv_dm_sep_t dm = c->dm;
    dm.rows = dm_rows_cur;
    rc = aoenv_shwfs_geometric(opd_a, nullptr, &dm, (const float*)c->pupil, (const float*)c->amp, (const int32_t*)c->valid_idx,
                               c->nV, c->B, c->nS, c->n, c->phase_scale, c->inv_units, (float*)c->slopes, c->lds,
                               tc ? c->slope_planes : nullptr, 2, (double*)c->stats, stream);
    if (rc) return rc;
  } else if (parts & 1) {
    aoenv_dm_sep_t dm = c->dm;
    dm.rows = dm_rows_cur;
    rc = aoenv_shwfs_frame_dm(opd_a, nullptr, &dm, (const int32_t*)c->order, (const float*)c->pupil, (const float*)c->amp,
                              (const uint8_t*)c->valid, c->B, c->nS, c->n, c->phase_scale, det, 0, (float*)c->frame,
                              (int32_t*)c->envmax, (double*)c->stats, stream);
    if (rc) return rc;
    rc = aoenv_shwfs_slopes((const float*)c->frame, (const int32_t*)c->envmax, 0, (const int32_t*)c->valid_idx, c->nV,
                            (const float*)c->ref_xy, c->inv_units, c->threshold_cog, c->B, c->nS, c->n, (float*)c->slopes, c->lds,
                            tc ? c->slope_planes : nullptr, 2, stream);
    if (rc) return rc;
  }
  if (parts & 2) {
    if (tc)
      rc = aoenv_gemm_tn_tc(c->slope_planes, c->rec_planes, c->lds, c->rec_parts, (float*)c->rec, c->ldr, c->B, c->nA, c->lds,
                            1.0f, stream);
    else
      rc = aoenv_gemm_tn((const float*)c->slopes, c->lds, (const float*)c->rec_f32, c->lds, (float*)c->rec, c->ldr, c->B, c->nA,
                         c->lds, 1.0f, stream);
    if (rc) return rc;
    rc = aoenv_observe((const float*)c->rec, c->ldr, (const int32_t*)c->act_idx, c->B, c->nA, c->nAct2, (const double*)c->stats,
                       c->n_pupil, c->phase_scale, obs, reward, strehl, total, residual, stream);
    if (rc) return rc;
  }
  if (parts & 4) {
    rc = aoenv_command_update(action, (const int32_t*)c->act_idx, c->B, c->nA, c->nAct2, c->leak, coefs_next, (float*)c->dm_prev,
                              c->ldc, stream);
    if (rc) return rc;
    rc = aoenv_dm_rows(coefs_next, c->ldc, (const int32_t*)c->act_pos, c->nA, c->nAct, c->dm.nActP, (const float*)c->wx,
                       (const int32_t*)c->j0x, c->W, c->B, c->nS * c->n, dm_rows_next, stream);
  }
  return rc;
}
```

### rlao_b200/csrc/wfs.cu

```cuda
#include <stdlib.h>
#include <mutex>

#include "common.cuh"
#include "wfs_twiddles.inc"

namespace aoenv {

constexpr int kMaxN = 8;
__constant__ float2 c_tw[2 * kMaxN * kMaxN];
__constant__ double2 c_twd[2 * kMaxN * kMaxN];
static int g_tw_n[64] = {0};
static std::mutex g_tw_mutex;

static int ensure_twiddles(int n, cudaStream_t stream) {
  int dev = 0;
  cudaGetDevice(&dev);
  std::lock_guard<std::mutex> lock(g_tw_mutex);
  if (dev < 64 && g_tw_n[dev] == n) return 0;
  const int N = 2 * n;
  float2 h[2 * kMaxN * kMaxN];
  double2 hd[2 * kMaxN * kMaxN];
  for (int u = 0; u < N; ++u)
    for (int a = 0; a < n; ++a) {
      const long m = ((long)(a + n / 2) * (2 * u + N + 1)) % (2L * N);
// ... 82 lines not shown
    return __logf(V * invalpha * __frcp_rn(__fdividef(a, us * us) + bb)) <= -lam + k * loglam - log_factorial(k);
  }
};
constexpr int kPtrsMaxAttempts = 15;

__device__ __forceinline__ float poisson_draw(float lam, uint32_t w0, uint32_t w1, const PixelRng& rng, uint32_t retry_block) {
  if (!(lam > 0.f)) return 0.f;
  if (lam < 12.f) return poisson_small_loop(lam, u32_to_unit(w0) * 0.99999994f);
  const Ptrs pt(lam);
  for (int it = 0; it < kPtrsMaxAttempts; ++it) {
    if (it > 0) {
      const uint4 r = rng.block(retry_block + (uint32_t)it);
      w0 = r.x;
      w1 = r.y;
    }
    float k;
    if (pt.attempt(w0, w1, k)) return k;
  }
  return rintf(lam);
}

__device__ __forceinline__ float detector_finish(float photons, float dark, float ron, const aoenv_detector_t& d, uint32_t stages) {
  float x = photons;
  if (stages & 1u) x *= d.qe;
  if (stages & 2u) {
    x += dark;
    if (d.has_fwc) x = fminf(fmaxf(x, 0.f), d.fwc);
    if (d.sensor_emccd) x *= d.gain;
  }
  if (stages & 4u) {
    x += ron;
    if (!d.sensor_emccd) x *= d.gain;
    if (d.bits > 0) {
      const float full = (float)((1u << d.bits) - 1u);
      x = truncf(x / d.fwc * full);
      x = fminf(x, full);
    }
  }
  return x;
}

constexpr int kDetPerLane = 8;
struct DetQueued { float lam, ron; uint32_t w0, w1; int pix; };

__device__ __forceinline__ uint32_t spare_word(const uint4& r) {
  return (r.x & 0xffu) | ((r.y & 0xffu) << 8) | ((r.z & 0xffu) << 16) | (r.w << 24);
}

__global__ void __launch_bounds__(256)
shwfs_detector_kernel(float* __restrict__ frame, const uint8_t* __restrict__ valid, int nS, int n, float inv_R, float inv_n,
                      const __grid_constant__ aoenv_detector_t det, int shared_max, int32_t* __restrict__ envmax,
                      int n_pixels) {
  pdl_enter();
  __shared__ DetQueued queue[8][kDetPerLane * 32];
  const int R = nS * n, P = n_pixels > 0 ? n_pixels : R * R;
  const int b = blockIdx.y, lane = threadIdx.x & 31, warp = threadIdx.x >> 5;
  const int first = (blockIdx.x * 8 + warp) * (kDetPerLane * 32);
  float* __restrict__ img = frame + (size_t)b * P;
  DetQueued* __restrict__ q = queue[warp];
  int queued = 0;
  float vmax = -INFINITY;
  const uint32_t stages = det.reserved ? det.reserved : 7u;
  const bool photon_noise = det.photon_noise && (stages & 1u);
  const bool has_dark = det.dark_electrons > 0.f && (stages & 2u);
  const bool has_ron = det.readout_noise != 0.f && (stages & 4u);
  const float dark_p0 = has_dark ? __expf(-det.dark_electrons) : 1.f;

  auto is_lit = [&](int pix) {
    if (valid == nullptr) return envmax != nullptr;
    const int y = (int)(((float)pix + 0.5f) * inv_R);
    const int x = pix - y * R;
    const int li = (int)(((float)y + 0.5f) * inv_n), lj = (int)(((float)x + 0.5f) * inv_n);
    return valid[li * nS + lj] != 0;
  };
  auto track = [&](int pix, float val) {
    if (val > vmax && is_lit(pix)) vmax = val;
  };
  auto dark_draw = [&](const uint4& r0, const PixelRng& rng) {
    if (!has_dark) return 0.f;
    const uint32_t w = spare_word(r0);
    const float u = u32_to_unit(w) * 0.99999994f;
    if (!(u > dark_p0)) return 0.f;
    if (det.dark_electrons < 12.f) return poisson_small_loop(det.dark_electrons, u);
    const uint4 r1 = rng.block(1);
    return poisson_draw(det.dark_electrons, r1.x, r1.y, rng, 32);
  };

#pragma unroll 2
  for (int j = 0; j < kDetPerLane; ++j) {
    const int pix = first + j * 32 + lane;
    const bool in = pix < P;
    const float lam = in ? img[pix] : 0.f;
    const PixelRng rng(det.seed, (uint32_t)pix, (uint32_t)b, det.frame_counter);
    const uint4 r0 = rng.block(0);
    float ron = 0.f;
    if (has_ron)
      ron = rintf(sqrtf(-2.0f * __logf(u32_to_unit(r0.z))) * __cosf(6.283185307179586f * u32_to_unit(r0.w)) * det.readout_noise);
    const float dark = dark_draw(r0, rng);
    const bool ptrs = in && photon_noise && lam >= 12.f;
    if (!ptrs && in) {
      const float photons = photon_noise ? poisson_small(lam, u32_to_unit(r0.x) * 0.99999994f) : lam;
      const float val = detector_finish(photons, dark, ron, det, stages);
      img[pix] = val;
      track(pix, val);
    }
    const unsigned m = __ballot_sync(0xffffffffu, ptrs);
    if (ptrs) {
      const uint32_t dk = (uint32_t)fminf(dark, 65535.f);
      q[queued + __popc(m & ((1u << lane) - 1u))] = {lam, ron, (r0.x & ~0xffu) | (dk & 0xffu), (r0.y & ~0xffu) | (dk >> 8), pix};
    }
    queued += __popc(m);
  }
  __syncwarp();
  for (int round = 0; queued > 0; ++round) {
    int kept = 0;
    for (int e0 = 0; e0 < queued; e0 += 32) {
      const int e = e0 + lane;
      const bool have = e < queued;
      DetQueued it = q[have ? e : 0];
      bool rejected = false;
      if (have) {
        const float dark = (float)((it.w0 & 0xffu) | ((it.w1 & 0xffu) << 8));
        if (round > 0) {
          const PixelRng rng(det.seed, (uint32_t)it.pix, (uint32_t)b, det.frame_counter);
          const uint4 r = rng.block(16u + (uint32_t)round);
          it.w0 = (r.x & ~0xffu) | (it.w0 & 0xffu);
          it.w1 = (r.y & ~0xffu) | (it.w1 & 0xffu);
        }
        const Ptrs pt(it.lam);
        float photons;
        bool ok = pt.attempt(it.w0, it.w1, photons);
        if (!ok && round == kPtrsMaxAttempts - 1) { photons = rintf(it.lam); ok = true; }
        if (ok) {
          const float val = detector_finish(photons, dark, it.ron, det, stages);
          img[it.pix] = val;
          track(it.pix, val);
        }
        rejected = !ok;
      }
      __syncwarp();
      const unsigned m = __ballot_sync(0xffffffffu, rejected);
      if (rejected) q[kept + __popc(m & ((1u << lane) - 1u))] = it;
      kept += __popc(m);
    }
    __syncwarp();
    queued = kept;
  }
  if (envmax != nullptr) {
    vmax = warp_max(vmax);
    if (lane == 0 && vmax > -INFINITY) atomicMax(&envmax[shared_max ? 0 : b], float_to_ordered(vmax));
  }
}

template <int n, int WL = 0>
__global__ void __launch_bounds__(128)
shwfs_frame_kernel(const float* __restrict__ opd_a, const float* __restrict__ opd_b, const float* __restrict__ pupil,
                   const float* __restrict__ amp, const uint8_t* __restrict__ valid, int nS, float phase_scale,
                   int track_max, int shared_max, float* __restrict__ frame,
                   int32_t* __restrict__ envmax, double* __restrict__ stats, const __grid_constant__ aoenv_dm_sep_t dm,
                   const int32_t* __restrict__ order) {
  constexpr int N = 2 * n;
  pdl_enter();
  const int R = nS * n;
  const int b = blockIdx.y;
  const int k0 = blockIdx.x * blockDim.x + threadIdx.x;
  const bool active = k0 < nS * nS;
  const int k = (active && order != nullptr) ? __ldg(&order[k0]) : k0;
  const int li = active ? k / nS : 0, lj = active ? k % nS : 0;
  const bool lit = active && valid[k] != 0;
  const float phase_turns = phase_scale * 0.15915494309189535f;

  float2 er2[n][n / 2], ei2[n][n / 2];
  float f0 = 0.f, f1 = 0.f, f2 = 0.f, f3 = 0.f;
  if (active) {
    const size_t tile = (size_t)(li * n) * R + lj * n;
    const float* __restrict__ pa = opd_a + (size_t)b * R * R + tile;
    const float* __restrict__ pb = (WL == 0 && opd_b) ? opd_b + (size_t)b * R * R + tile : nullptr;
    const size_t centre = (size_t)b * R * R + (size_t)(R / 2) * R + R / 2;
    const float ka = stats ? __ldg(opd_a + centre) : 0.f;
    const float kt = stats ? (pb ? ka + __ldg(opd_b + centre) : ka) : 0.f;
    float2 dmv[WL > 0 ? n : 1][n / 2];
    if (WL > 0) {
      constexpr int half = (WL + 1) / 2, hp = (half + 3) / 4 * 4;
#pragma unroll
      for (int bb = 0; bb < n; ++bb)
#pragma unroll
        for (int a2 = 0; a2 < n / 2; ++a2) dmv[WL > 0 ? bb : 0][a2] = make_float2(0.f, 0.f);
      const float* __restrict__ trow = dm.rows + ((size_t)b * dm.nActP + __ldg(&dm.ilr[li])) * R + lj * n;
      const float* __restrict__ wrow = dm.wlr + (size_t)(li * n) * (2 * hp);
#pragma unroll
      for (int g = 0; g < 2 * hp / 4; ++g) {
        float4 w4[n];
#pragma unroll
        for (int bb = 0; bb < n; ++bb) w4[bb] = __ldg(reinterpret_cast<const float4*>(wrow + (size_t)bb * (2 * hp)) + g);
#pragma unroll
        for (int e = 0; e < 4; ++e) {
          const int j = 4 * g + e, hh = j / hp, kk = j % hp;
          if (kk >= half) continue;
          const int t = hh * half + kk;
          if (t >= WL) continue;
          float2 tv[n / 2];
#pragma unroll
          for (int a2 = 0; a2 < n / 2; ++a2) tv[a2] = __ldg(reinterpret_cast<const float2*>(trow + (size_t)t * R) + a2);
#pragma unroll
          for (int bb = 0; bb < n; ++bb) {
            const float w = e == 0 ? w4[bb].x : (e == 1 ? w4[bb].y : (e == 2 ? w4[bb].z : w4[bb].w));
#pragma unroll
            for (int a2 = 0; a2 < n / 2; ++a2) dmv[WL > 0 ? bb : 0][a2] = fma2(dup2(w), tv[a2], dmv[WL > 0 ? bb : 0][a2]);
          }
        }
      }
    }
#pragma unroll
    for (int bb = 0; bb < n; ++bb) {
#pragma unroll
      for (int a2 = 0; a2 < n / 2; ++a2) {
        const int o2 = bb * R + 2 * a2;
        const float2 av = __ldg(reinterpret_cast<const float2*>(pa + o2));
        const float2 bv = WL > 0 ? dmv[WL > 0 ? bb : 0][a2]
                                 : (pb ? __ldg(reinterpret_cast<const float2*>(pb + o2)) : make_float2(0.f, 0.f));
        const float2 pv = __ldg(reinterpret_cast<const float2*>(pupil + tile + o2));
        const float2 mv = lit ? __ldg(reinterpret_cast<const float2*>(amp + tile + o2)) : make_float2(0.f, 0.f);
#pragma unroll
        for (int e = 0; e < 2; ++e) {
          const int aa = 2 * a2 + e;
          const float a = e ? av.y : av.x;
          const float t = a + (e ? bv.y : bv.x);
          const float pu = e ? pv.y : pv.x;
          const float in_pupil = pu > 0.f ? 1.f : 0.f;
          const float da = (a - ka) * in_pupil, dt = (t - kt) * in_pupil;
          f0 += da; f1 = fmaf(da, da, f1); f2 += dt; f3 = fmaf(dt, dt, f3);
          const float turns = t * pu * phase_turns;
          const float ang = (turns - ((turns + 12582912.0f) - 12582912.0f)) * 6.283185307179586f;
          const float sn = __sinf(ang), cs = __cosf(ang);
          const float am = e ? mv.y : mv.x;
          if ((bb & 1) == 0) { er2[aa][bb >> 1].x = am * cs; ei2[aa][bb >> 1].x = am * sn; }
          else { er2[aa][bb >> 1].y = am * cs; ei2[aa][bb >> 1].y = am * sn; }
        }
      }
    }
  }
  double s0 = (double)f0, s1 = (double)f1, s2 = (double)f2, s3 = (double)f3;

  if (stats != nullptr) {
    s0 = warp_sum(s0); s1 = warp_sum(s1); s2 = warp_sum(s2); s3 = warp_sum(s3);
    if ((threadIdx.x & 31) == 0) {
      double* __restrict__ st = stats + (size_t)b * 4;
      atomicAdd(st, s0); atomicAdd(st + 1, s1); atomicAdd(st + 2, s2); atomicAdd(st + 3, s3);
    }
  }

  float vmax = -INFINITY;
  if (active) {
    float* __restrict__ fout = frame + (size_t)b * R * R + (size_t)(li * n) * R + lj * n;
    const float norm = 1.0f / (float)(N * N);
    constexpr int h = n / 2;
#pragma unroll 1
    for (int pp = 0; pp < h; ++pp) {
      float2 acc[n];
#pragma unroll
      for (int q = 0; q < n; ++q) acc[q] = make_float2(0.f, 0.f);
      if (lit) {
#pragma unroll
        for (int du = 0; du < 2; ++du) {
          const int u = 2 * pp + du;
          float2 pr[h], pi[h], qr[h], qi[h];
#pragma unroll
          for (int k = 0; k < h; ++k) { pr[k] = pi[k] = qr[k] = qi[k] = make_float2(0.f, 0.f); }
#pragma unroll
          for (int aa = 0; aa < n; ++aa) {
            const float2 g = c_tw[u * n + aa];
            const float2 gx = dup2(g.x), gy = dup2(g.y), ngy = dup2(-g.y);
            if (((aa + h) & 1) == 0) {
#pragma unroll
              for (int k = 0; k < h; ++k) {
                pr[k] = fma2(gx, er2[aa][k], fma2(ngy, ei2[aa][k], pr[k]));
                pi[k] = fma2(gx, ei2[aa][k], fma2(gy, er2[aa][k], pi[k]));
              }
            } else {
#pragma unroll
              for (int k = 0; k < h; ++k) {
                qr[k] = fma2(gx, er2[aa][k], fma2(ngy, ei2[aa][k], qr[k]));
                qi[k] = fma2(gx, ei2[aa][k], fma2(gy, er2[aa][k], qi[k]));
              }
            }
          }
          float2 yr[n], yi[n];
#pragma unroll
          for (int bb = 0; bb < n; ++bb) {
            const float p_r = (bb & 1) ? pr[bb >> 1].y : pr[bb >> 1].x, q_r = (bb & 1) ? qr[bb >> 1].y : qr[bb >> 1].x;
            const float p_i = (bb & 1) ? pi[bb >> 1].y : pi[bb >> 1].x, q_i = (bb & 1) ? qi[bb >> 1].y : qi[bb >> 1].x;
            yr[bb] = make_float2(p_r + q_r, p_r - q_r);
            yi[bb] = make_float2(p_i + q_i, p_i - q_i);
          }
#pragma unroll
          for (int v = 0; v < n; ++v) {
            float2 er_ = make_float2(0.f, 0.f), ei_ = er_, or_ = er_, oi_ = er_;
#pragma unroll
            for (int bb = 0; bb < n; ++bb) {
              const float gx = WfsTw<n>::re(v * n + bb), gy = WfsTw<n>::im(v * n + bb);
              if (((bb + h) & 1) == 0) {
                er_ = fma2(yr[bb], dup2(gx), fma2(yi[bb], dup2(-gy), er_));
                ei_ = fma2(yr[bb], dup2(gy), fma2(yi[bb], dup2(gx), ei_));
              } else {
                or_ = fma2(yr[bb], dup2(gx), fma2(yi[bb], dup2(-gy), or_));
                oi_ = fma2(yr[bb], dup2(gy), fma2(yi[bb], dup2(gx), oi_));
              }
            }
            const float2 f0r = add2(er_, or_), f0i = add2(ei_, oi_);
            const float2 f1r = sub2(er_, or_), f1i = sub2(ei_, oi_);
            acc[v >> 1] = add2(acc[v >> 1], fma2(f0r, f0r, mul2(f0i, f0i)));
            acc[(v >> 1) + h] = add2(acc[(v >> 1) + h], fma2(f1r, f1r, mul2(f1i, f1i)));
          }
        }
      }
#pragma unroll
      for (int r2 = 0; r2 < 2; ++r2) {
        const int p = pp + r2 * h;
#pragma unroll
        for (int q = 0; q < n; ++q) {
          const float val = (r2 == 0 ? acc[q].x : acc[q].y) * norm;
          fout[(size_t)p * R + q] = val;
          if (lit) vmax = fmaxf(vmax, val);
        }
      }
    }
  }
  if (track_max) {
    vmax = warp_max(vmax);
    if ((threadIdx.x & 31) == 0 && vmax > -INFINITY) atomicMax(&envmax[shared_max ? 0 : b], float_to_ordered(vmax));
  }
}

struct C2 { float2 r, i; };
__device__ __forceinline__ C2 cadd(const C2& a, const C2& b) { return {add2(a.r, b.r), add2(a.i, b.i)}; }
__device__ __forceinline__ C2 csub(const C2& a, const C2& b) { return {sub2(a.r, b.r), sub2(a.i, b.i)}; }
__device__ __forceinline__ C2 cmulc(const C2& a, float wr, float wi) {
  return {fma2(a.r, dup2(wr), mul2(a.i, dup2(-wi))), fma2(a.r, dup2(wi), mul2(a.i, dup2(wr)))};
}
__device__ __forceinline__ void dft3(const C2& z0, const C2& z1, const C2& z2, C2& y0, C2& y1, C2& y2) {
  constexpr float c = 0.8660254037844386f;
  const C2 t = cadd(z1, z2), d = csub(z1, z2);
  y0 = cadd(z0, t);
  const C2 m = {fma2(dup2(-0.5f), t.r, z0.r), fma2(dup2(-0.5f), t.i, z0.i)};
  y1 = {fma2(dup2(c), d.i, m.r), fma2(dup2(-c), d.r, m.i)};
  y2 = {fma2(dup2(-c), d.i, m.r), fma2(dup2(c), d.r, m.i)};
}
template <int K1>
__device__ __forceinline__ void dft6_half(const C2 (&z)[6], C2& y0, C2& y1, C2& y2) {
  const C2 s0 = K1 == 0 ? cadd(z[0], z[3]) : csub(z[0], z[3]);
  const C2 s1 = K1 == 0 ? cadd(z[2], z[5]) : csub(z[2], z[5]);
  const C2 s2 = K1 == 0 ? cadd(z[4], z[1]) : csub(z[4], z[1]);
  dft3(s0, s1, s2, y0, y1, y2);
}
__device__ __forceinline__ void twiddle6(const C2 (&z)[6], C2 (&w)[6]) {
  constexpr float c = 0.8660254037844386f;
  w[0] = z[0];
  w[1] = cmulc(z[1], c, -0.5f);
  w[2] = cmulc(z[2], 0.5f, -c);
  w[3] = {z[3].i, mul2(z[3].r, dup2(-1.0f))};
  w[4] = cmulc(z[4], -0.5f, -c);
  w[5] = cmulc(z[5], -c, -0.5f);
}
__host__ __device__ constexpr int dft6_row(int k1, int k2) { return (3 * k1 + 4 * k2) % 6; }

template <int K1>
__device__ __forceinline__ void wfs6_pass1(const float* __restrict__ sF, C2 (&Hp)[3][6]) {
  constexpr float c = 0.8660254037844386f;
#pragma unroll
  for (int b = 0; b < 6; ++b) {
    C2 z[6];
#pragma unroll
    for (int a = 0; a < 6; ++a) {
      const float xr = sF[(2 * (a * 6 + b)) * 128], xi = sF[(2 * (a * 6 + b) + 1) * 128];
      float wr, wi;
      if (a == 0) { wr = xr; wi = xi; }
      else if (a == 1) { wr = fmaf(xr, c, xi * 0.5f); wi = fmaf(xi, c, xr * -0.5f); }
      else if (a == 2) { wr = fmaf(xr, 0.5f, xi * c); wi = fmaf(xi, 0.5f, xr * -c); }
      else if (a == 3) { wr = xi; wi = -xr; }
      else if (a == 4) { wr = fmaf(xr, -0.5f, xi * c); wi = fmaf(xi, -0.5f, xr * -c); }
      else { wr = fmaf(xr, -c, xi * 0.5f); wi = fmaf(xi, -c, xr * -0.5f); }
      z[a] = {make_float2(xr, wr), make_float2(xi, wi)};
    }
    dft6_half<K1>(z, Hp[0][b], Hp[1][b], Hp[2][b]);
  }
}

template <int K1>
__device__ __forceinline__ void wfs6_pass2(const C2 (&Hp)[3][6], float norm, float* __restrict__ fout, int R, float& vmax) {
#pragma unroll
  for (int k2 = 0; k2 < 3; ++k2) {
    const int p = dft6_row(K1, k2);
    C2 yw[6];
    twiddle6(Hp[k2], yw);
    float row[6];
#pragma unroll
    for (int q1 = 0; q1 < 2; ++q1) {
      C2 e[3], o[3];
      if (q1 == 0) { dft6_half<0>(Hp[k2], e[0], e[1], e[2]); dft6_half<0>(yw, o[0], o[1], o[2]); }
      else { dft6_half<1>(Hp[k2], e[0], e[1], e[2]); dft6_half<1>(yw, o[0], o[1], o[2]); }
#pragma unroll
      for (int q2 = 0; q2 < 3; ++q2) {
        const float2 i0 = fma2(e[q2].r, e[q2].r, mul2(e[q2].i, e[q2].i));
        const float2 i1 = fma2(o[q2].r, o[q2].r, mul2(o[q2].i, o[q2].i));
        const float2 t = add2(i0, i1);
        row[dft6_row(q1, q2)] = (t.x + t.y) * norm;
      }
    }
#pragma unroll
    for (int q = 0; q < 6; ++q) {
      fout[(size_t)p * R + q] = row[q];
      vmax = fmaxf(vmax, row[q]);
    }
  }
}

__global__ void __launch_bounds__(128, 3)
shwfs_frame6_kernel(const float* __restrict__ opd_a, const float* __restrict__ opd_b, const float* __restrict__ pupil,
                    const float* __restrict__ amp, const uint8_t* __restrict__ valid, int nS, float phase_scale,
                    int track_max, int shared_max, float* __restrict__ frame, int32_t* __restrict__ envmax,
                    double* __restrict__ stats) {
  constexpr int n = 6, N = 12;
  __shared__ float sF_all[2 * n * n * 128];
  float* __restrict__ sF = sF_all + threadIdx.x;
  const int R = nS * n;
  const int b = blockIdx.y;
  const int k = blockIdx.x * blockDim.x + threadIdx.x;
  const bool active = k < nS * nS;
  const int li = active ? k / nS : 0, lj = active ? k % nS : 0;
  const bool lit = active && valid[k] != 0;
  const float phase_turns = phase_scale * 0.15915494309189535f;
  float f0 = 0.f, f1 = 0.f, f2 = 0.f, f3 = 0.f;
  if (active) {
    const size_t tile = (size_t)(li * n) * R + lj * n;
    const float* __restrict__ pa = opd_a + (size_t)b * R * R + tile;
    const float* __restrict__ pb = opd_b ? opd_b + (size_t)b * R * R + tile : nullptr;
    const size_t centre = (size_t)b * R * R + (size_t)(R / 2) * R + R / 2;
    const float ka = stats ? __ldg(opd_a + centre) : 0.f;
    const float kt = stats ? (opd_b ? ka + __ldg(opd_b + centre) : ka) : 0.f;
#pragma unroll
    for (int bb = 0; bb < n; ++bb) {
#pragma unroll
      for (int aa = 0; aa < n; ++aa) {
        const int o = bb * R + aa;
        const float a = __ldg(pa + o);
        const float t = pb ? a + __ldg(pb + o) : a;
        const float pu = __ldg(pupil + tile + o);
        const float in_pupil = pu > 0.f ? 1.f : 0.f;
        const float da = (a - ka) * in_pupil, dt = (t - kt) * in_pupil;
        f0 += da; f1 = fmaf(da, da, f1); f2 += dt; f3 = fmaf(dt, dt, f3);
        if (lit) {
          constexpr double kTurn = -13.0 / 24.0;
          const double cst = kTurn * (double)(aa + bb + n);
          const float cfrac = (float)(cst - (double)(long long)(cst - 0.5));
          const float turns = fmaf(t * pu, phase_turns, cfrac);
          const float ang = (turns - ((turns + 12582912.0f) - 12582912.0f)) * 6.283185307179586f;
          const float am = __ldg(amp + tile + o);
          sF[(2 * (aa * n + bb)) * 128] = am * __cosf(ang);
          sF[(2 * (aa * n + bb) + 1) * 128] = am * __sinf(ang);
        }
      }
    }
  }
  if (stats != nullptr) {
    double s0 = warp_sum((double)f0), s1 = warp_sum((double)f1), s2 = warp_sum((double)f2), s3 = warp_sum((double)f3);
    if ((threadIdx.x & 31) == 0) {
      double* __restrict__ st = stats + (size_t)b * 4;
      atomicAdd(st, s0); atomicAdd(st + 1, s1); atomicAdd(st + 2, s2); atomicAdd(st + 3, s3);
    }
  }
  float vmax = -INFINITY;
  if (active) {
    float* __restrict__ fout = frame + (size_t)b * R * R + (size_t)(li * n) * R + lj * n;
    if (lit) {
      const float norm = 1.0f / (float)(N * N);
      C2 Hp[3][6];
      wfs6_pass1<0>(sF, Hp);
      wfs6_pass2<0>(Hp, norm, fout, R, vmax);
      wfs6_pass1<1>(sF, Hp);
      wfs6_pass2<1>(Hp, norm, fout, R, vmax);
    } else {
#pragma unroll
      for (int p = 0; p < n; ++p)
// ... 173 lines not shown
  const float phase_turns = phase_scale * 0.15915494309189535f;
  const size_t tile = (size_t)(li * n) * R + lj * n;
  float f0 = 0.f, f1 = 0.f, f2 = 0.f, f3 = 0.f;
  float2 er2[n], ei2[n];
  if (active) {
    const float* __restrict__ pa = opd_a + (size_t)b * R * R + tile;
    const float* __restrict__ pb = opd_b ? opd_b + (size_t)b * R * R + tile : nullptr;
    const size_t centre = (size_t)b * R * R + (size_t)(R / 2) * R + R / 2;
    const float ka = stats ? __ldg(opd_a + centre) : 0.f;
    const float kt = stats ? (opd_b ? ka + __ldg(opd_b + centre) : ka) : 0.f;
#pragma unroll
    for (int e = 0; e < 2; ++e) {
      const int bb = 2 * t + e;
#pragma unroll
      for (int a2 = 0; a2 < h; ++a2) {
        const int o2 = bb * R + 2 * a2;
        const float2 av = __ldg(reinterpret_cast<const float2*>(pa + o2));
        const float2 bv = pb ? __ldg(reinterpret_cast<const float2*>(pb + o2)) : make_float2(0.f, 0.f);
        const float2 pv = __ldg(reinterpret_cast<const float2*>(pupil + tile + o2));
        const float2 mv = lit ? __ldg(reinterpret_cast<const float2*>(amp + tile + o2)) : make_float2(0.f, 0.f);
#pragma unroll
        for (int h2 = 0; h2 < 2; ++h2) {
          const int aa = 2 * a2 + h2;
          const float a = h2 ? av.y : av.x;
          const float tt = a + (h2 ? bv.y : bv.x);
          const float pu = h2 ? pv.y : pv.x;
          const float in_pupil = pu > 0.f ? 1.f : 0.f;
          const float da = (a - ka) * in_pupil, dt = (tt - kt) * in_pupil;
          f0 += da; f1 = fmaf(da, da, f1); f2 += dt; f3 = fmaf(dt, dt, f3);
          const float turns = tt * pu * phase_turns;
          const float ang = (turns - ((turns + 12582912.0f) - 12582912.0f)) * 6.283185307179586f;
          const float am = h2 ? mv.y : mv.x;
          const float cs = am * __cosf(ang), sn = am * __sinf(ang);
          if (e == 0) { er2[aa].x = cs; ei2[aa].x = sn; } else { er2[aa].y = cs; ei2[aa].y = sn; }
        }
      }
    }
  }
  if (stats != nullptr) {
    double s0 = warp_sum((double)f0), s1 = warp_sum((double)f1), s2 = warp_sum((double)f2), s3 = warp_sum((double)f3);
    if (lane == 0) {
      double* __restrict__ st = stats + (size_t)b * 4;
      atomicAdd(st, s0); atomicAdd(st + 1, s1); atomicAdd(st + 2, s2); atomicAdd(st + 3, s3);
    }
  }
  float2 (*x)[S] = xch[warp];
  const bool any_lit = __any_sync(0xffffffffu, lit);
  float vmax = -INFINITY;
  if (any_lit) {
    if (lit) {
#pragma unroll
      for (int u = 0; u < n; ++u) {
        float2 pr = make_float2(0.f, 0.f), pi = pr, qr = pr, qi = pr;
#pragma unroll
        for (int aa = 0; aa < n; ++aa) {
          const float gx = WfsTw<n>::re(u * n + aa), gy = WfsTw<n>::im(u * n + aa);
          if (((aa + h) & 1) == 0) {
            pr = fma2(dup2(gx), er2[aa], fma2(dup2(-gy), ei2[aa], pr));
            pi = fma2(dup2(gx), ei2[aa], fma2(dup2(gy), er2[aa], pi));
          } else {
            qr = fma2(dup2(gx), er2[aa], fma2(dup2(-gy), ei2[aa], qr));
            qi = fma2(dup2(gx), ei2[aa], fma2(dup2(gy), er2[aa], qi));
          }
        }
        x[(0 * T + t) * n + u][slot] = pr;
        x[(1 * T + t) * n + u][slot] = pi;
        x[(2 * T + t) * n + u][slot] = qr;
        x[(3 * T + t) * n + u][slot] = qi;
      }
    }
    __syncwarp();
    if (lit) {
      float* __restrict__ fout = frame + (size_t)b * R * R + tile;
      const float norm = 1.0f / (float)(N * N);
      float2 acc[n];
#pragma unroll
      for (int q = 0; q < n; ++q) acc[q] = make_float2(0.f, 0.f);
#pragma unroll
      for (int du = 0; du < 2; ++du) {
        const int u = 2 * t + du;
        float2 yr[n], yi[n];
#pragma unroll
        for (int kk = 0; kk < T; ++kk) {
          const float2 pr = x[(0 * T + kk) * n + u][slot], pi = x[(1 * T + kk) * n + u][slot];
          const float2 qr = x[(2 * T + kk) * n + u][slot], qi = x[(3 * T + kk) * n + u][slot];
          yr[2 * kk] = make_float2(pr.x + qr.x, pr.x - qr.x);
          yr[2 * kk + 1] = make_float2(pr.y + qr.y, pr.y - qr.y);
          yi[2 * kk] = make_float2(pi.x + qi.x, pi.x - qi.x);
          yi[2 * kk + 1] = make_float2(pi.y + qi.y, pi.y - qi.y);
        }
#pragma unroll
        for (int v = 0; v < n; ++v) {
          float2 er_ = make_float2(0.f, 0.f), ei_ = er_, or_ = er_, oi_ = er_;
#pragma unroll
          for (int bb = 0; bb < n; ++bb) {
            const float gx = WfsTw<n>::re(v * n + bb), gy = WfsTw<n>::im(v * n + bb);
            if (((bb + h) & 1) == 0) {
              er_ = fma2(yr[bb], dup2(gx), fma2(yi[bb], dup2(-gy), er_));
              ei_ = fma2(yr[bb], dup2(gy), fma2(yi[bb], dup2(gx), ei_));
            } else {
              or_ = fma2(yr[bb], dup2(gx), fma2(yi[bb], dup2(-gy), or_));
              oi_ = fma2(yr[bb], dup2(gy), fma2(yi[bb], dup2(gx), oi_));
            }
          }
          const float2 f0r = add2(er_, or_), f0i = add2(ei_, oi_);
          const float2 f1r = sub2(er_, or_), f1i = sub2(ei_, oi_);
          acc[v >> 1] = add2(acc[v >> 1], fma2(f0r, f0r, mul2(f0i, f0i)));
          acc[(v >> 1) + h] = add2(acc[(v >> 1) + h], fma2(f1r, f1r, mul2(f1i, f1i)));
        }
      }
#pragma unroll
      for (int q2 = 0; q2 < h; ++q2) {
        const float2 lo = make_float2(acc[2 * q2].x * norm, acc[2 * q2 + 1].x * norm);
        const float2 hi = make_float2(acc[2 * q2].y * norm, acc[2 * q2 + 1].y * norm);
        *reinterpret_cast<float2*>(fout + (size_t)t * R + 2 * q2) = lo;
        *reinterpret_cast<float2*>(fout + (size_t)(t + h) * R + 2 * q2) = hi;
        vmax = fmaxf(vmax, fmaxf(fmaxf(lo.x, lo.y), fmaxf(hi.x, hi.y)));
      }
    }
  }
  if (active && !lit) {
    float* __restrict__ fout = frame + (size_t)b * R * R + tile;
#pragma unroll
    for (int e = 0; e < 2; ++e)
#pragma unroll
      for (int q2 = 0; q2 < h; ++q2) *reinterpret_cast<float2*>(fout + (size_t)(2 * t + e) * R + 2 * q2) = make_float2(0.f, 0.f);
  }
  if (track_max) {
    vmax = warp_max(vmax);
    if (lane == 0 && vmax > -INFINITY) atomicMax(&envmax[shared_max ? 0 : b], float_to_ordered(vmax));
  }
}

template <int n>
__global__ void __launch_bounds__(128)
shwfs_slopes_kernel(const float* __restrict__ frame, const int32_t* __restrict__ envmax, int shared_max,
                    const int32_t* __restrict__ valid_idx, int nV, const float* __restrict__ ref_xy, float inv_units,
                    float threshold_cog, int nS, float* __restrict__ slopes, int lds,
                    __nv_bfloat16* __restrict__ planes, int parts) {
  const int b = blockIdx.y;
  pdl_enter();
  const int t = blockIdx.x * blockDim.x + threadIdx.x;
  if (t >= nV) return;
  const int R = nS * n;
  const int k = __ldg(&valid_idx[t]);
  const int li = k / nS, lj = k - li * nS;
  const float thr = threshold_cog * ordered_to_float(__ldg(&envmax[shared_max ? 0 : b]));
  const float* __restrict__ f = frame + (size_t)b * R * R + (size_t)(li * n) * R + lj * n;
  float2 v[n][n / 2];
#pragma unroll
  for (int p = 0; p < n; ++p)
#pragma unroll
    for (int h = 0; h < n / 2; ++h) v[p][h] = __ldg(reinterpret_cast<const float2*>(f + (size_t)p * R) + h);
  float s = 0.f, sx = 0.f, sy = 0.f;
#pragma unroll
  for (int p = 0; p < n; ++p)
#pragma unroll
    for (int q = 0; q < n; ++q) {
      float x = (q & 1) ? v[p][q >> 1].y : v[p][q >> 1].x;
      x = x < thr ? 0.f : x;
      s += x;
      sx = fmaf(x, (float)p, sx);
      sy = fmaf(x, (float)q, sy);
    }
  float cx = sx / s, cy = sy / s;
  if (!isfinite(cx)) cx = 0.f;
  if (!isfinite(cy)) cy = 0.f;
  const float sx_ = (cx - __ldg(&ref_xy[t])) * inv_units, sy_ = (cy - __ldg(&ref_xy[nV + t])) * inv_units;
  slopes[(size_t)b * lds + t] = sx_;
  slopes[(size_t)b * lds + nV + t] = sy_;
  if (planes != nullptr) {
    store_bf16_planes(planes, (size_t)gridDim.y * lds, (size_t)b * lds + t, parts, sx_);
    store_bf16_planes(planes, (size_t)gridDim.y * lds, (size_t)b * lds + nV + t, parts, sy_);
  }
}

template <int n>
__global__ void __launch_bounds__(64)
shwfs_frame_f64_kernel(const float* __restrict__ opd, const float* __restrict__ pupil, const float* __restrict__ amp,
                       const uint8_t* __restrict__ valid, int nS, double phase_scale, int shared_max,
                       double* __restrict__ frame, unsigned long long* __restrict__ envmax) {
  constexpr int N = 2 * n;
  const int R = nS * n;
  const int b = blockIdx.y;
  const int k = blockIdx.x * blockDim.x + threadIdx.x;
  if (k >= nS * nS) return;
  const int li = k / nS, lj = k % nS;
  const bool lit = valid[k] != 0;
  const size_t tile = (size_t)(li * n) * R + lj * n;
  double* __restrict__ fout = frame + (size_t)b * R * R + tile;
  if (!lit) {
    for (int p = 0; p < n; ++p)
      for (int q = 0; q < n; ++q) fout[(size_t)p * R + q] = 0.0;
    return;
  }
  double er[n][n], ei[n][n];
  const float* __restrict__ pa = opd + (size_t)b * R * R + tile;
#pragma unroll
  for (int bb = 0; bb < n; ++bb)
#pragma unroll
    for (int aa = 0; aa < n; ++aa) {
      const int o = bb * R + aa;
      double sn, cs;
      sincos((double)__ldg(pa + o) * (double)__ldg(pupil + tile + o) * phase_scale, &sn, &cs);
      const double am = (double)__ldg(amp + tile + o);
      er[aa][bb] = am * cs;
      ei[aa][bb] = am * sn;
    }
  double vmax = 0.0;
  const double norm = 1.0 / (double)(N * N);
  for (int p = 0; p < n; ++p) {
    double acc[n];
#pragma unroll
    for (int q = 0; q < n; ++q) acc[q] = 0.0;
    for (int du = 0; du < 2; ++du) {
      const int u = 2 * p + du;
      double yr[n], yi[n];
#pragma unroll
      for (int bb = 0; bb < n; ++bb) { yr[bb] = 0.0; yi[bb] = 0.0; }
#pragma unroll
      for (int aa = 0; aa < n; ++aa) {
        const double2 g = c_twd[u * n + aa];
#pragma unroll
        for (int bb = 0; bb < n; ++bb) {
          yr[bb] += g.x * er[aa][bb] - g.y * ei[aa][bb];
          yi[bb] += g.x * ei[aa][bb] + g.y * er[aa][bb];
        }
      }
#pragma unroll
      for (int v = 0; v < N; ++v) {
        double fr = 0.0, fi = 0.0;
#pragma unroll
        for (int bb = 0; bb < n; ++bb) {
          const double2 g = c_twd[v * n + bb];
          fr += yr[bb] * g.x - yi[bb] * g.y;
          fi += yr[bb] * g.y + yi[bb] * g.x;
        }
        acc[v >> 1] += fr * fr + fi * fi;
      }
    }
#pragma unroll
    for (int q = 0; q < n; ++q) {
      const double val = acc[q] * norm;
      fout[(size_t)p * R + q] = val;
      vmax = fmax(vmax, val);
    }
  }
  atomicMax(&envmax[shared_max ? 0 : b], (unsigned long long)__double_as_longlong(vmax));
}

__global__ void __launch_bounds__(128)
shwfs_slopes_f64_kernel(const double* __restrict__ frame, const unsigned long long* __restrict__ envmax, int shared_max,
                        const int32_t* __restrict__ valid_idx, int nV, const double* __restrict__ ref_xy,
                        double inv_units, double threshold_cog, int nS, int n, double* __restrict__ slopes, int lds) {
  const int b = blockIdx.y;
  const int t = blockIdx.x * blockDim.x + threadIdx.x;
  if (t >= nV) return;
  const int R = nS * n;
  const int k = __ldg(&valid_idx[t]);
  const int li = k / nS, lj = k % nS;
  const double thr = threshold_cog * __longlong_as_double((long long)envmax[shared_max ? 0 : b]);
  const double* __restrict__ f = frame + (size_t)b * R * R + (size_t)(li * n) * R + lj * n;
  double s = 0.0, sx = 0.0, sy = 0.0;
  for (int p = 0; p < n; ++p)
    for (int q = 0; q < n; ++q) {
      double v = f[(size_t)p * R + q];
      v = v < thr ? 0.0 : v;
      s += v;
      sx += v * (double)p;
      sy += v * (double)q;
    }
  double cx = sx / s, cy = sy / s;
  if (!isfinite(cx)) cx = 0.0;
  if (!isfinite(cy)) cy = 0.0;
  slopes[(size_t)b * lds + t] = (cx - ref_xy[t]) * inv_units;
  slopes[(size_t)b * lds + nV + t] = (cy - ref_xy[nV + t]) * inv_units;
}

__global__ void envmax_init_kernel(int32_t* __restrict__ envmax, int count, double* __restrict__ stats, int n_stats) {
  pdl_enter();
  const int i = blockIdx.x * blockDim.x + threadIdx.x;
  if (i < count) envmax[i] = float_to_ordered(-INFINITY);
  if (stats != nullptr && i < n_stats) stats[i] = 0.0;
}

}

using namespace aoenv;

constexpr int kDefaultFrameVariant = 0;
static std::atomic<int> g_wfs6_factorised{[] {
  const char* e = getenv("AOENV_WFS_FRAME");
  if (e && e[0] == 'f') return 1;
  if (e && e[0] == 's') return (e[5] == '6') ? 2 : 3;
  if (e && e[0] == 't') return 0;
  return kDefaultFrameVariant;
}()};

extern "C" {

int aoenv_set_wfs6_variant(int variant) {
  return g_wfs6_factorised.exchange(variant < 0 || variant > 3 ? kDefaultFrameVariant : variant);
}

static int shwfs_frame_impl(const float* opd_a, const float* opd_b, const aoenv_dm_sep_t* dm_in, const int32_t* order, const float* pupil,
                            const float* amp, const uint8_t* valid, int B, int nS, int n, float phase_scale,
                            const aoenv_detector_t* det, int shared_max, float* frame, int32_t* envmax, double* stats,
                            void* stream) {
  AOENV_CHECK_ARG(B > 0 && B <= 65535 && nS > 0, "shwfs_frame: bad shape B=%d nS=%d", B, nS);
  aoenv_dm_sep_t dm{};
  if (dm_in != nullptr) {
    dm = *dm_in;
    AOENV_CHECK_ARG(opd_b == nullptr, "shwfs_frame_dm: give either the separable DM or an explicit second OPD term");
    AOENV_CHECK_ARG(dm.rows != nullptr && dm.wlr != nullptr && dm.ilr != nullptr && dm.nActP > 0, "shwfs_frame_dm: bad DM tables");
    AOENV_CHECK_ARG(dm.WL == 14 || dm.WL == 18, "shwfs_frame_dm: DM window of %d actuator rows (14 or 18)", dm.WL);
    AOENV_CHECK_ARG((reinterpret_cast<uintptr_t>(dm.rows) & 7) == 0 && (reinterpret_cast<uintptr_t>(dm.wlr) & 15) == 0,
                    "shwfs_frame_dm: DM tables must be 16-byte aligned");
  }
  AOENV_CHECK_ARG(n == 4 || n == 6 || n == 8, "shwfs_frame: %d pixels per lenslet is not a compiled size (4, 6, 8)", n);
  cudaStream_t s = (cudaStream_t)stream;
  if (det) {
    AOENV_CHECK_ARG(!(det->bits > 0 && !det->has_fwc), "shwfs_frame: ADC without a full-well capacity is not supported");
    AOENV_CHECK_ARG(det->bits >= 0 && det->bits < 31, "shwfs_frame: bits=%d", det->bits);
  }
  int rc = ensure_twiddles(n, s);
  if (rc) return rc;
  AOENV_LAUNCH(envmax_init_kernel, dim3((4 * B + 255) / 256), 256, 0, s, envmax, shared_max ? 1 : B, stats, stats ? 4 * B : 0);
  AOENV_LAUNCH_CHECK("envmax_init");
  dim3 grid((nS * nS + 127) / 128, B);
  const int variant = g_wfs6_factorised.load(std::memory_order_relaxed);
  if (variant == 3 && dm.WL == 0) {
    const int per_block = 4 * (32 / (n / 2));
    dim3 g3((nS * nS + per_block - 1) / per_block, B);
    if (n == 4) shwfs_frame_split_kernel<4><<<g3, 128, 0, s>>>(opd_a, opd_b, pupil, amp, valid, nS, phase_scale, det == nullptr, shared_max, frame, envmax, stats);
    else if (n == 6) shwfs_frame_split_kernel<6><<<g3, 128, 0, s>>>(opd_a, opd_b, pupil, amp, valid, nS, phase_scale, det == nullptr, shared_max, frame, envmax, stats);
    else shwfs_frame_split_kernel<8><<<g3, 128, 0, s>>>(opd_a, opd_b, pupil, amp, valid, nS, phase_scale, det == nullptr, shared_max, frame, envmax, stats);
  } else
#define AOENV_WFS_CASE(NN)                                                                                   \
  case NN:                                                                                                   \
    if (dm.WL == 14)                                                                                         \
      AOENV_LAUNCH((shwfs_frame_kernel<NN, 14>), grid, 128, 0, s, opd_a, opd_b, pupil, amp, valid, nS, phase_scale, \
                   (int)(det == nullptr), shared_max, frame, envmax, stats, dm, order);                             \
    else if (dm.WL == 18)                                                                                    \
      AOENV_LAUNCH((shwfs_frame_kernel<NN, 18>), grid, 128, 0, s, opd_a, opd_b, pupil, amp, valid, nS, phase_scale, \
                   (int)(det == nullptr), shared_max, frame, envmax, stats, dm, order);                             \
    else                                                                                                     \
      AOENV_LAUNCH((shwfs_frame_kernel<NN, 0>), grid, 128, 0, s, opd_a, opd_b, pupil, amp, valid, nS, phase_scale,  \
                   (int)(det == nullptr), shared_max, frame, envmax, stats, dm, order);                             \
    break;
  switch (n) {
    AOENV_WFS_CASE(4)
    AOENV_WFS_CASE(8)
    case 6:
      if (dm.WL != 0) {
        if (dm.WL == 14) {
          AOENV_LAUNCH((shwfs_frame_kernel<6, 14>), grid, 128, 0, s, opd_a, opd_b, pupil, amp, valid, nS, phase_scale,
                       (int)(det == nullptr), shared_max, frame, envmax, stats, dm, order);
        } else
          AOENV_LAUNCH((shwfs_frame_kernel<6, 18>), grid, 128, 0, s, opd_a, opd_b, pupil, amp, valid, nS, phase_scale,
                       (int)(det == nullptr), shared_max, frame, envmax, stats, dm, order);
      } else if (variant == 2) {
        dim3 g3((nS * nS + kS6Warps * kS6Lenslets - 1) / (kS6Warps * kS6Lenslets), B);
        shwfs_frame6s_kernel<<<g3, kS6Warps * 32, 0, s>>>(opd_a, opd_b, pupil, amp, valid, nS, phase_scale, det == nullptr,
                                                          shared_max, frame, envmax, stats);
      } else if (variant == 1)
        shwfs_frame6_kernel<<<grid, 128, 0, s>>>(opd_a, opd_b, pupil, amp, valid, nS, phase_scale, det == nullptr, shared_max,
                                                 frame, envmax, stats);
      else
        AOENV_LAUNCH((shwfs_frame_kernel<6, 0>), grid, 128, 0, s, opd_a, opd_b, pupil, amp, valid, nS, phase_scale,
                     (int)(det == nullptr), shared_max, frame, envmax, stats, dm, order);
      break;
  }
#undef AOENV_WFS_CASE
  AOENV_LAUNCH_CHECK("shwfs_frame");
  if (det) {
    const int R = nS * n;
    AOENV_CHECK_ARG(R * R < (1 << 24), "shwfs_frame: frame of %d x %d pixels is too large for the camera pass", R, R);
    dim3 gd((R * R + 8 * kDetPerLane * 32 - 1) / (8 * kDetPerLane * 32), B);
    AOENV_LAUNCH(shwfs_detector_kernel, gd, 256, 0, s, frame, valid, nS, n, 1.0f / (float)R, 1.0f / (float)n, *det, shared_max, envmax, 0);
    AOENV_LAUNCH_CHECK("shwfs_detector");
  }
  return 0;
}

int aoenv_shwfs_frame(const float* opd_a, const float* opd_b, const float* pupil, const float* amp,
                      const uint8_t* valid, int B, int nS, int n, float phase_scale, const aoenv_detector_t* det,
                      int shared_max, float* frame, int32_t* envmax, double* stats, void* stream) {
  return shwfs_frame_impl(opd_a, opd_b, nullptr, nullptr, pupil, amp, valid, B, nS, n, phase_scale, det, shared_max, frame, envmax, stats, stream);
}

int aoenv_shwfs_frame_dm(const float* opd_a, const float* opd_b, const aoenv_dm_sep_t* dm, const int32_t* order,
                         const float* pupil, const float* amp, const uint8_t* valid, int B, int nS, int n, float phase_scale,
                         const aoenv_detector_t* det, int shared_max, float* frame, int32_t* envmax, double* stats,
                         void* stream) {
  return shwfs_frame_impl(opd_a, opd_b, dm, order, pupil, amp, valid, B, nS, n, phase_scale, det, shared_max, frame, envmax, stats, stream);
}

int aoenv_shwfs_camera(float* frame, const uint8_t* valid, int B, int nS, int n, const aoenv_detector_t* det, int shared_max,
                       int32_t* envmax, void* stream) {
  AOENV_CHECK_ARG(B > 0 && B <= 65535 && nS > 0 && n > 0, "shwfs_camera: bad shape B=%d nS=%d", B, nS);
  AOENV_CHECK_ARG(det != nullptr && valid != nullptr && envmax != nullptr, "shwfs_camera: detector, lenslet mask and envmax are required");
  AOENV_CHECK_ARG(!(det->bits > 0 && !det->has_fwc), "shwfs_camera: ADC without a full-well capacity is not supported");
  AOENV_CHECK_ARG(det->bits >= 0 && det->bits < 31, "shwfs_camera: bits=%d", det->bits);
  const int R = nS * n;
  AOENV_CHECK_ARG(R * R < (1 << 24), "shwfs_camera: frame of %d x %d pixels is too large for the camera pass", R, R);
  cudaStream_t s = (cudaStream_t)stream;
  AOENV_LAUNCH(envmax_init_kernel, dim3((B + 255) / 256), 256, 0, s, envmax, shared_max ? 1 : B, (double*)nullptr, 0);
  AOENV_LAUNCH_CHECK("envmax_init");
  dim3 gd((R * R + 8 * kDetPerLane * 32 - 1) / (8 * kDetPerLane * 32), B);
  shwfs_detector_kernel<<<gd, 256, 0, s>>>(frame, valid, nS, n, 1.0f / (float)R, 1.0f / (float)n, *det, shared_max, envmax, 0);
  AOENV_LAUNCH_CHECK("shwfs_detector");
  return 0;
}

int aoenv_detector_integrate(float* frame, int B, int rows, int cols, const aoenv_detector_t* det, void* stream) {
  AOENV_CHECK_ARG(B > 0 && B <= 65535 && rows > 0 && cols > 0 && (long long)rows * cols < (1 << 24), "detector_integrate: bad shape");
  AOENV_CHECK_ARG(det != nullptr, "detector_integrate: no detector given");
  AOENV_CHECK_ARG(!(det->bits > 0 && !det->has_fwc), "detector_integrate: ADC without a full-well capacity is not supported");
  AOENV_CHECK_ARG(det->bits >= 0 && det->bits < 31, "detector_integrate: bits=%d", det->bits);
  const int P = rows * cols;
  dim3 gd((P + 8 * kDetPerLane * 32 - 1) / (8 * kDetPerLane * 32), B);
  shwfs_detector_kernel<<<gd, 256, 0, (cudaStream_t)stream>>>(frame, nullptr, 1, 1, 1.0f, 1.0f, *det, 0, nullptr, P);
  AOENV_LAUNCH_CHECK("detector_integrate");
  return 0;
}

int aoenv_shwfs_slopes(const float* frame, const int32_t* envmax, int shared_max, const int32_t* valid_idx, int nV,
                       const float* ref_xy, float inv_units, float threshold_cog, int B, int nS, int n, float* slopes,
                       int lds, void* slope_planes, int parts, void* stream) {
  AOENV_CHECK_ARG(B > 0 && B <= 65535 && nV > 0 && lds >= 2 * nV, "shwfs_slopes: bad shape B=%d nV=%d lds=%d", B, nV, lds);
  AOENV_CHECK_ARG(n == 4 || n == 6 || n == 8, "shwfs_slopes: %d pixels per lenslet is not a compiled size (4, 6, 8)", n);
  AOENV_CHECK_ARG((reinterpret_cast<uintptr_t>(frame) & 7) == 0, "shwfs_slopes: frame must be 8-byte aligned");
  dim3 grid((nV + 127) / 128, B);
#define AOENV_SLOPES_CASE(NN)                                                                                          \
  case NN:                                                                                                             \
    AOENV_LAUNCH(shwfs_slopes_kernel<NN>, grid, 128, 0, (cudaStream_t)stream, frame, envmax, shared_max, valid_idx, nV, \
                 ref_xy, inv_units, threshold_cog, nS, slopes, lds, (__nv_bfloat16*)slope_planes, parts);              \
    break;
  switch (n) {
    AOENV_SLOPES_CASE(4)
    AOENV_SLOPES_CASE(6)
    AOENV_SLOPES_CASE(8)
  }
#undef AOENV_SLOPES_CASE
  AOENV_LAUNCH_CHECK("shwfs_slopes");
  return 0;
}

int aoenv_shwfs_measure_f64(const float* opd, const float* pupil, const float* amp, const uint8_t* valid,
                            const int32_t* valid_idx, int nV, const double* ref_xy, double inv_units, double threshold_cog,
                            int F, int nS, int n, double phase_scale, int shared_max, double* frame, uint64_t* envmax,
                            double* slopes, int lds, void* stream) {
  AOENV_CHECK_ARG(F > 0 && F <= 65535 && nS > 0 && nV > 0 && lds >= 2 * nV, "shwfs_measure_f64: bad shape");
  AOENV_CHECK_ARG(n == 4 || n == 6 || n == 8, "shwfs_measure_f64: %d pixels per lenslet is not a compiled size (4, 6, 8)", n);
  cudaStream_t s = (cudaStream_t)stream;
  int rc = ensure_twiddles(n, s);
  if (rc) return rc;
  cudaError_t e = cudaMemsetAsync(envmax, 0, sizeof(uint64_t) * (shared_max ? 1 : (size_t)F), s);
  if (e != cudaSuccess) return fail(-3, "shwfs_measure_f64 memset: %s", cudaGetErrorString(e));
  dim3 grid((nS * nS + 63) / 64, F);
  unsigned long long* em = reinterpret_cast<unsigned long long*>(envmax);
  switch (n) {
    case 4: shwfs_frame_f64_kernel<4><<<grid, 64, 0, s>>>(opd, pupil, amp, valid, nS, phase_scale, shared_max, frame, em); break;
    case 6: shwfs_frame_f64_kernel<6><<<grid, 64, 0, s>>>(opd, pupil, amp, valid, nS, phase_scale, shared_max, frame, em); break;
    case 8: shwfs_frame_f64_kernel<8><<<grid, 64, 0, s>>>(opd, pupil, amp, valid, nS, phase_scale, shared_max, frame, em); break;
  }
  AOENV_LAUNCH_CHECK("shwfs_frame_f64");
  dim3 g2((nV + 127) / 128, F);
  shwfs_slopes_f64_kernel<<<g2, 128, 0, s>>>(frame, em, shared_max, valid_idx, nV, ref_xy, inv_units, threshold_cog, nS, n,
                                             slopes, lds);
  AOENV_LAUNCH_CHECK("shwfs_slopes_f64");
  return 0;
}

}
```

### rlao_b200/csrc/wfs_fused.cu

```cuda
#include <cooperative_groups.h>

#include "common.cuh"
#include "tma.cuh"
#include "wfs_twiddles.inc"

namespace cg = cooperative_groups;

namespace aoenv {

constexpr int kMaxCluster = 16;
__host__ __device__ constexpr int wl_half(int WL) { return (WL + 1) / 2; }
__host__ __device__ constexpr int wl_half_pad(int WL) { return (wl_half(WL) + 3) & ~3; }
__host__ __device__ constexpr int wl_stride(int WL) { return 2 * wl_half_pad(WL); }

struct FusedArgs {
  const float* opd_a;
  const float* opd_b;
  aoenv_dm_sep_t dm;
  const uint8_t* pupil8;
  const int32_t* order;
  const int32_t* nlit;
  const int32_t* slot_of;
  const float* ref_xy;
  float amp0, phase_scale, inv_units, threshold_cog;
// ... 266 lines not shown
                                      (m[r] & 0xff000000u) ? 1.f : 0.f);
        ma.add(a, in);
        mt.add(t, in);
        cnt += (in.x + in.y) + (in.z + in.w);
      }
    }
    if (p.stats != nullptr) {
      const double dca = (double)ma.c, dct = (double)mt.c, dn = (double)cnt;
      A1 += (double)ma.s1 + dn * dca;
      A2 += (double)ma.s2 + 2.0 * dca * (double)ma.s1 + dn * dca * dca;
      T1 += (double)mt.s1 + dn * dct;
      T2 += (double)mt.s2 + 2.0 * dct * (double)mt.s1 + dn * dct * dct;
    }
  }
  if (p.stats != nullptr) {
    A1 = warp_sum(A1); A2 = warp_sum(A2); T1 = warp_sum(T1); T2 = warp_sum(T2);
    if (lane == 0) { misc->warp_stats[warp][0] = A1; misc->warp_stats[warp][1] = A2; misc->warp_stats[warp][2] = T1; misc->warp_stats[warp][3] = T2; }
  }
  __syncthreads();

  const int g = warp / T, part = warp - g * T;
  const int LPC = rows * nS;
  const int nlit = __ldg(&p.nlit[rank]);
  const int32_t* __restrict__ order = p.order + (size_t)rank * p.rows_max * nS;
  float2* const F = Fall + (size_t)g * (n * n * 32) + lane;
  const float phase_turns = p.phase_scale * 0.15915494309189535f;
  const float norm = 1.0f / (float)(N * N);
  float vmax = -INFINITY;
  for (int c0 = g * 32; c0 < LPC; c0 += NG * 32) {
    const int idx = c0 + lane;
    const bool lit = idx < nlit;
    const int lens = idx < LPC ? __ldg(&order[idx]) : 0;
    const int lr = lens / nS, l = lens - lr * nS;
    const int cbase = (lr * n) * HP + l * h;
    const bool any_lit = c0 < nlit;
    if (any_lit) {
      if (lit) {
        float2 rowv[2][h];
        uint32_t rowm[2][h];
#pragma unroll
        for (int e = 0; e < 2; ++e)
#pragma unroll
          for (int a2 = 0; a2 < h; ++a2) {
            rowv[e][a2] = S2[cbase + (2 * part + e) * HP + a2];
            rowm[e][a2] = mask16[cbase + (2 * part + e) * HP + a2];
          }
#pragma unroll
        for (int aa = 0; aa < n; ++aa) {
          float re[2], im[2];
#pragma unroll
          for (int e = 0; e < 2; ++e) {
            const float t = (aa & 1) ? rowv[e][aa >> 1].y : rowv[e][aa >> 1].x;
            const bool in = ((rowm[e][aa >> 1] >> ((aa & 1) * 8)) & 0xffu) != 0;
            const float turns = t * phase_turns;
            const float ang = (turns - ((turns + 12582912.0f) - 12582912.0f)) * 6.283185307179586f;
            const float am = in ? p.amp0 : 0.f;
            re[e] = am * __cosf(ang);
            im[e] = am * __sinf(ang);
          }
          F[fidx<n>(aa, part, 0)] = make_float2(re[0], re[1]);
          F[fidx<n>(aa, part, 1)] = make_float2(im[0], im[1]);
        }
      }
      group_bar(1 + g, T * 32);
    }
    if (idx < LPC) {
      float2 acc[n];
      if (lit) {
        spot_rows_dispatch<n>(part, F, acc);
      } else {
#pragma unroll
        for (int q = 0; q < n; ++q) acc[q] = make_float2(0.f, 0.f);
      }
#pragma unroll
      for (int q2 = 0; q2 < h; ++q2) {
        const float2 lo = make_float2(acc[2 * q2].x * norm, acc[2 * q2 + 1].x * norm);
        const float2 hi = make_float2(acc[2 * q2].y * norm, acc[2 * q2 + 1].y * norm);
        S2[cbase + part * HP + q2] = lo;
        S2[cbase + (part + h) * HP + q2] = hi;
        if (lit) vmax = fmaxf(vmax, fmaxf(fmaxf(lo.x, lo.y), fmaxf(hi.x, hi.y)));
      }
    }
    if (any_lit) group_bar(1 + g, T * 32);
  }

  vmax = warp_max(vmax);
  if (lane == 0) misc->warp_max[warp] = vmax;
  if (p.frame != nullptr) {
    asm volatile("fence.proxy.async.shared::cta;" ::: "memory");
  }
  __syncthreads();
  if (tid < C) {
    float m = -INFINITY;
    for (int w = 0; w < kThreads / 32; ++w) m = fmaxf(m, misc->warp_max[w]);
    *cluster.map_shared_rank(&misc->peer_max[rank], tid) = m;
  } else if (p.stats != nullptr && tid >= 32 && tid < 36) {
    const int k = tid - 32;
    double s = 0.0;
    for (int w = 0; w < kThreads / 32; ++w) s += misc->warp_stats[w][k];
    *cluster.map_shared_rank(&misc->peer_stats[rank][k], 0) = s;
  }
  if (p.frame != nullptr && tid == 64) {
    char* dst = reinterpret_cast<char*>(p.frame + env_off + (size_t)row0_px * R);
    for (uint32_t o = 0; o < strip_bytes; o += 32768u)
      bulk_store(dst + o, reinterpret_cast<const char*>(S) + o, min(32768u, strip_bytes - o));
    asm volatile("cp.async.bulk.commit_group;" ::: "memory");
  }
  cluster.sync();
  if (tid == 0) {
    float m = -INFINITY;
    for (int r = 0; r < C; ++r) m = fmaxf(m, misc->peer_max[r]);
    misc->env_max = m;
    if (rank == 0 && p.envmax != nullptr) p.envmax[b] = float_to_ordered(p.do_slopes ? m : -INFINITY);
  }
  if (p.stats != nullptr && rank == 0 && tid >= 32 && tid < 36) {
    double s = 0.0;
    for (int r = 0; r < C; ++r) s += misc->peer_stats[r][tid - 32];
    p.stats[(size_t)b * 4 + (tid - 32)] = s;
  }
  __syncthreads();
  if (p.do_slopes) {
    const float thr = p.threshold_cog * misc->env_max;
    const size_t plane_stride = (size_t)gridDim.y * p.lds;
    for (int idx = tid; idx < nlit; idx += kThreads) {
      const int lens = __ldg(&order[idx]);
      const int lr = lens / nS, l = lens - lr * nS;
      const int cbase = (lr * n) * HP + l * h;
      float s = 0.f, sx = 0.f, sy = 0.f;
#pragma unroll
      for (int pr_ = 0; pr_ < n; ++pr_)
#pragma unroll
        for (int q2 = 0; q2 < h; ++q2) {
          const float2 v = S2[cbase + pr_ * HP + q2];
          const float x0 = v.x < thr ? 0.f : v.x, x1 = v.y < thr ? 0.f : v.y;
          s += x0; sx = fmaf(x0, (float)pr_, sx); sy = fmaf(x0, (float)(2 * q2), sy);
          s += x1; sx = fmaf(x1, (float)pr_, sx); sy = fmaf(x1, (float)(2 * q2 + 1), sy);
        }
      float cx = sx / s, cy = sy / s;
      if (!isfinite(cx)) cx = 0.f;
      if (!isfinite(cy)) cy = 0.f;
      const int t = __ldg(&p.slot_of[(lr0 + lr) * nS + l]);
      const float sx_ = (cx - __ldg(&p.ref_xy[t])) * p.inv_units, sy_ = (cy - __ldg(&p.ref_xy[p.nV + t])) * p.inv_units;
      p.slopes[(size_t)b * p.lds + t] = sx_;
      p.slopes[(size_t)b * p.lds + p.nV + t] = sy_;
      if (p.planes != nullptr) {
        store_bf16_planes(p.planes, plane_stride, (size_t)b * p.lds + t, p.parts, sx_);
        store_bf16_planes(p.planes, plane_stride, (size_t)b * p.lds + p.nV + t, p.parts, sy_);
      }
    }
  }
  if (p.frame != nullptr && tid == 64) asm volatile("cp.async.bulk.wait_group.read 0;" ::: "memory");
}

template <int W>
__global__ void __launch_bounds__(256)
dm_rows_kernel(const float* __restrict__ coefs, int ldc, const int32_t* __restrict__ act_pos, int nA, int nAct, int nActP,
               const float* __restrict__ wx, const int32_t* __restrict__ j0x, int R, float* __restrict__ rows) {
  pdl_enter();
  extern __shared__ __align__(16) float sC[];
  const int b = blockIdx.x, ldC = nAct + W;
  for (int k = threadIdx.x; k < nAct * ldC; k += blockDim.x) sC[k] = 0.f;
  __syncthreads();
  for (int k = threadIdx.x; k < nA; k += blockDim.x) {
    const int pos = __ldg(&act_pos[k]);
    const int r = pos / nAct;
    sC[r * ldC + (pos - r * nAct)] = __ldg(&coefs[(size_t)b * ldc + k]);
  }
  __syncthreads();
  float* __restrict__ out = rows + (size_t)b * nActP * R;
  for (int x = threadIdx.x; x < R; x += blockDim.x) {
    float w[W];
    const int j0 = __ldg(&j0x[x]);
#pragma unroll
    for (int q = 0; q < W / 4; ++q) {
      const float4 v = __ldg(reinterpret_cast<const float4*>(wx + (size_t)x * W) + q);
      w[4 * q] = v.x; w[4 * q + 1] = v.y; w[4 * q + 2] = v.z; w[4 * q + 3] = v.w;
    }
    const int per = (nAct + gridDim.y - 1) / gridDim.y;
    const int i_lo = blockIdx.y * per, i_hi = min(nAct, i_lo + per);
#pragma unroll 4
    for (int i = i_lo; i < i_hi; ++i) {
      const float* __restrict__ c = sC + i * ldC + j0;
      float t = 0.f;
#pragma unroll
      for (int q = 0; q < W; ++q) t = fmaf(c[q], w[q], t);
      out[(size_t)i * R + x] = t;
    }
  }
}

template <int n, int NG, int WL>
static int launch_fused(const FusedArgs& a, int B, int C, size_t smem, cudaStream_t s) {
  auto kern = shwfs_fused_kernel<n, NG, WL>;
  cudaError_t e = cudaFuncSetAttribute(kern, cudaFuncAttributeMaxDynamicSharedMemorySize, (int)smem);
  if (e == cudaSuccess && C > 8) e = cudaFuncSetAttribute(kern, cudaFuncAttributeNonPortableClusterSizeAllowed, 1);
  if (e != cudaSuccess) return fail(-3, "shwfs_fused attributes: %s", cudaGetErrorString(e));
  cudaLaunchConfig_t cfg = {};
  cfg.gridDim = dim3(C, B, 1);
  cfg.blockDim = dim3(NG * (n / 2) * 32, 1, 1);
  cfg.dynamicSmemBytes = smem;
  cfg.stream = s;
  cudaLaunchAttribute attr[1];
  attr[0].id = cudaLaunchAttributeClusterDimension;
  attr[0].val.clusterDim.x = C;
  attr[0].val.clusterDim.y = 1;
  attr[0].val.clusterDim.z = 1;
  cfg.attrs = attr;
  cfg.numAttrs = 1;
  e = cudaLaunchKernelEx(&cfg, kern, a);
  if (e != cudaSuccess) return fail(-3, "shwfs_fused launch (cluster %d, %zu B shared): %s", C, smem, cudaGetErrorString(e));
  return 0;
}

}

using namespace aoenv;

extern "C" {

int aoenv_shwfs_fused_smem(int nS, int n, int rows_max, int groups, int t_rows, int WL) {
  if (nS <= 0 || rows_max <= 0 || rows_max > nS || (n != 4 && n != 6 && n != 8)) return -1;
  return fused_smem_layout(nS, n, rows_max, groups, t_rows, WL > 0 ? WL : 14, t_rows > 0).total;
}

int aoenv_dm_rows(const float* coefs, int ldc, const int32_t* act_pos, int nA, int nAct, int nActP, const float* wx,
                  const int32_t* j0x, int W, int B, int R, float* rows, void* stream) {
  AOENV_CHECK_ARG(B > 0 && R > 0 && nAct > 0 && nA > 0 && nA <= nAct * nAct && ldc >= nA && nActP >= nAct, "dm_rows: bad shape");
  AOENV_CHECK_ARG(W == 12 || W == 16, "dm_rows: band width %d (12 or 16)", W);
  const size_t smem = (size_t)nAct * (nAct + W) * sizeof(float);
  AOENV_CHECK_ARG(smem <= 200 * 1024, "dm_rows: %d actuators across do not fit in shared memory", nAct);
  cudaStream_t s = (cudaStream_t)stream;
  cudaError_t e = W == 12 ? cudaFuncSetAttribute(dm_rows_kernel<12>, cudaFuncAttributeMaxDynamicSharedMemorySize, (int)smem)
                          : cudaFuncSetAttribute(dm_rows_kernel<16>, cudaFuncAttributeMaxDynamicSharedMemorySize, (int)smem);
  if (e != cudaSuccess) return fail(-3, "dm_rows smem attribute: %s", cudaGetErrorString(e));
  const dim3 grid(B, 1);
  if (W == 12) AOENV_LAUNCH(dm_rows_kernel<12>, grid, 256, smem, s, coefs, ldc, act_pos, nA, nAct, nActP, wx, j0x, R, rows);
  else AOENV_LAUNCH(dm_rows_kernel<16>, grid, 256, smem, s, coefs, ldc, act_pos, nA, nAct, nActP, wx, j0x, R, rows);
  AOENV_LAUNCH_CHECK("dm_rows");
  return 0;
}

int aoenv_shwfs_fused(const float* opd_a, const float* opd_b, const aoenv_dm_sep_t* dm, const uint8_t* pupil8, float amp0,
                      const int32_t* h_row_start, const int32_t* order, const int32_t* nlit, const int32_t* slot_of, int B,
                      int nS, int n, int cluster, int groups, float phase_scale, const float* ref_xy, int nV, float inv_units,
                      float threshold_cog, float* frame, float* slopes, int lds, void* slope_planes, int parts,
                      int32_t* envmax, double* stats, void* stream) {
  AOENV_CHECK_ARG(B > 0 && B <= 65535 && nS > 0, "shwfs_fused: bad shape B=%d nS=%d", B, nS);
  AOENV_CHECK_ARG(n == 4 || n == 6 || n == 8, "shwfs_fused: %d pixels per lenslet is not a compiled size (4, 6, 8)", n);
  AOENV_CHECK_ARG((nS * n) % 4 == 0, "shwfs_fused: the pupil must be a multiple of 4 pixels across (got %d)", nS * n);
  AOENV_CHECK_ARG(cluster >= 1 && cluster <= kMaxCluster && cluster <= nS, "shwfs_fused: cluster=%d out of range (1..%d)", cluster, kMaxCluster);
  AOENV_CHECK_ARG(groups >= 1 && groups <= 8, "shwfs_fused: groups=%d warp groups per CTA", groups);
  AOENV_CHECK_ARG(slopes == nullptr || (lds >= 2 * nV && nV > 0 && ref_xy != nullptr && slot_of != nullptr), "shwfs_fused: bad slopes arguments");
  AOENV_CHECK_ARG(slope_planes == nullptr || parts == 2 || parts == 3, "shwfs_fused: parts must be 2 or 3");
  AOENV_CHECK_ARG(slopes != nullptr || frame != nullptr, "shwfs_fused: neither slopes nor frame requested");
  AOENV_CHECK_ARG(h_row_start != nullptr && h_row_start[0] == 0 && h_row_start[cluster] == nS, "shwfs_fused: row_start must run from 0 to nS");
  const bool sep = dm != nullptr && dm->rows != nullptr;
  int WL = 14;
  if (sep) {
    AOENV_CHECK_ARG(dm->WL == 14 || dm->WL == 18, "shwfs_fused: DM window of %d actuator rows (14 or 18)", dm->WL);
    AOENV_CHECK_ARG(opd_b == nullptr, "shwfs_fused: give either the separable DM or an explicit second OPD term");
    AOENV_CHECK_ARG(dm->t_rows >= dm->WL && dm->nActP > 0 && dm->wlr != nullptr && dm->ilr != nullptr, "shwfs_fused: bad DM tables");
    WL = dm->WL;
  }
  FusedArgs a{};
  a.opd_a = opd_a; a.opd_b = opd_b;
  if (sep) a.dm = *dm;
  a.pupil8 = pupil8; a.order = order; a.nlit = nlit; a.slot_of = slot_of; a.ref_xy = ref_xy;
  a.amp0 = amp0; a.phase_scale = phase_scale; a.inv_units = inv_units; a.threshold_cog = threshold_cog;
  a.frame = frame; a.slopes = slopes; a.planes = (__nv_bfloat16*)slope_planes; a.envmax = envmax; a.stats = stats;
  a.lds = lds; a.parts = parts; a.nV = nV; a.nS = nS; a.do_slopes = slopes != nullptr;
  int rows_max = 0;
  for (int r = 0; r < cluster; ++r) {
    const int rows = h_row_start[r + 1] - h_row_start[r];
    AOENV_CHECK_ARG(rows >= 1, "shwfs_fused: strip %d is empty", r);
    rows_max = rows > rows_max ? rows : rows_max;
    a.row_start[r] = h_row_start[r];
  }
  a.row_start[cluster] = nS;
  a.rows_max = rows_max;
  const FusedSmem L = fused_smem_layout(nS, n, rows_max, groups, sep ? dm->t_rows : 0, WL, sep);
  AOENV_CHECK_ARG(L.total <= 227 * 1024, "shwfs_fused: %d bytes of shared memory per CTA (cluster %d): use a larger cluster", L.total, cluster);
  cudaStream_t s = (cudaStream_t)stream;
  int rc = -2;
#define AOENV_FUSED_CASE(NN, GG, WW) \
  if (n == NN && groups == GG && WL == WW) rc = launch_fused<NN, GG, WW>(a, B, cluster, (size_t)L.total, s);
  AOENV_FUSED_CASE(4, 4, 14) AOENV_FUSED_CASE(4, 4, 18)
  AOENV_FUSED_CASE(6, 2, 14) AOENV_FUSED_CASE(6, 4, 14) AOENV_FUSED_CASE(6, 4, 18) AOENV_FUSED_CASE(6, 6, 14)
  AOENV_FUSED_CASE(8, 4, 14) AOENV_FUSED_CASE(8, 4, 18)
  if (rc == -2) return fail(-2, "shwfs_fused: no kernel compiled for n=%d groups=%d WL=%d", n, groups, WL);
#undef AOENV_FUSED_CASE
  if (rc != 0) return rc;
  g_launches.fetch_add(1, std::memory_order_relaxed);
  return 0;
}

}
```

Before: 1.408 million.

## Fuse slope extraction into SH frame kernel and command update into DM rows

Adds a per-environment arrival counter so the last CTA of the Shack-Hartmann frame kernel computes centroid slopes in place, removing a separate slopes launch and frame reread from a cold kernel. It also folds the leaky-integrator command update into the DM row-building kernel, so coefficients are computed and placed into shared memory without a separate command kernel. Both paths are on by default behind an environment toggle. In exchange, the slopes tail runs serially in one CTA per environment and adds a release/acquire atomic handshake.

```diff
diff --git a/include/aoenv.h b/include/aoenv.h
--- a/include/aoenv.h
+++ b/include/aoenv.h
@@ -171,11 +171,13 @@
   const void* act_idx;
   void* dm_prev;
   const void *act_pos, *wx, *j0x;
+  void* arrivals;
 } aoenv_sh_step_t;
 
 int aoenv_sh_step(const aoenv_sh_step_t* c, int parts, const float* opd_a, const float* dm_rows_cur, const aoenv_detector_t* det,
                   const float* action, float* coefs_next, float* dm_rows_next, float* obs, float* reward, float* strehl,
                   float* total, float* residual, void* stream);
+int aoenv_set_sh_fuse(int enabled);
 
 int aoenv_shwfs_measure_f64(const float* opd, const float* pupil, const float* amp, const uint8_t* valid,
                             const int32_t* valid_idx, int nV, const double* ref_xy, double inv_units, double threshold_cog,
diff --git a/rlao_b200/OOPAOEnv/OOPAOEnvRazor.py b/rlao_b200/OOPAOEnv/OOPAOEnvRazor.py
--- a/rlao_b200/OOPAOEnv/OOPAOEnvRazor.py
+++ b/rlao_b200/OOPAOEnv/OOPAOEnvRazor.py
@@ -297,7 +297,8 @@
             c.amp, c.frame = wfs._flux.data_ptr(), None
             keep.append(wfs._flux)
         else:
-            c.frame = wfs._frame.data_ptr()
+            c.frame, c.arrivals = wfs._frame.data_ptr(), wfs._arrivals.data_ptr()
+            keep.append(wfs._arrivals)
         c.stats, c.slopes, c.slope_planes = wfs._stats.data_ptr(), wfs._signal.data_ptr(), wfs._signal_planes.data_ptr()
         c.dm.wlr, c.dm.ilr, c.dm.nActP, c.dm.WL = win[2].data_ptr(), win[1].data_ptr(), dm._rows.shape[2], win[0]
         c.rec_planes = self._Rm_op.planes().data_ptr() if tc else None
diff --git a/rlao_b200/ShackHartmann.py b/rlao_b200/ShackHartmann.py
--- a/rlao_b200/ShackHartmann.py
+++ b/rlao_b200/ShackHartmann.py
@@ -69,6 +69,7 @@
         B = self.n_envs
         self._frame = None if self._is_geometric else torch.zeros((B, R, R), dtype=torch.float32, device=self.device)
         self._envmax = torch.zeros((B,), dtype=torch.int32, device=self.device)
+        self._arrivals = torch.zeros((B,), dtype=torch.int32, device=self.device)
         self._stats = torch.zeros((B, 4), dtype=torch.float64, device=self.device)
         self._signal = torch.zeros((B, self._lds), dtype=torch.float32, device=self.device)
         self._signal_planes = torch.zeros((2, B, self._lds), dtype=torch.bfloat16, device=self.device)
diff --git a/rlao_b200/_lib.py b/rlao_b200/_lib.py
--- a/rlao_b200/_lib.py
+++ b/rlao_b200/_lib.py
@@ -44,7 +44,7 @@
         ("n_pupil", C.c_double)] + [(k, C.c_void_p) for k in ("pupil", "amp", "valid", "order", "valid_idx", "ref_xy", "frame",
                                                               "envmax", "stats", "slopes", "slope_planes")] + [
         ("dm", DmSepStruct)] + [(k, C.c_void_p) for k in ("rec_planes", "rec_f32", "rec", "act_idx", "dm_prev", "act_pos",
-                                                           "wx", "j0x")]
+                                                           "wx", "j0x", "arrivals")]
 
 
 class AtmState(C.Structure):
@@ -80,6 +80,7 @@
     "aoenv_gemm_tn_tc": [_vp, _vp, _i, _i, _vp, _i, _i, _i, _i, _f, _vp],
     "aoenv_dm_surface_separable": [_vp, _i, _vp, _i, _i, _vp, _vp, _vp, _vp, _vp, _vp, _vp, _vp, _i, _i, _i, _vp, _vp],
     "aoenv_set_wfs6_variant": [_i],
+    "aoenv_set_sh_fuse": [_i],
     "aoenv_detector_integrate": [_vp, _i, _i, _i, _vp, _vp],
     "aoenv_shwfs_camera": [_vp, _vp, _i, _i, _i, _vp, _i, _vp, _vp],
     "aoenv_shwfs_frame": [_vp, _vp, _vp, _vp, _vp, _i, _i, _i, _f, _vp, _i, _vp, _vp, _vp, _vp],
diff --git a/rlao_b200/csrc/common.cuh b/rlao_b200/csrc/common.cuh
--- a/rlao_b200/csrc/common.cuh
+++ b/rlao_b200/csrc/common.cuh
@@ -152,4 +152,33 @@
   }
 }
 
+__device__ __forceinline__ float command_value(float action, float dm_prev, float leak) {
+  const float act = action * 1e-6f;
+  return dm_prev * leak + act;
 }
+
+struct SlopesTail {
+  int32_t* arrivals;
+  const int32_t* valid_idx;
+  const float* ref_xy;
+  float* slopes;
+  __nv_bfloat16* planes;
+  float inv_units, threshold_cog;
+  int nV, lds, parts;
+};
+int shwfs_frame_dm_slopes(const float* opd_a, const aoenv_dm_sep_t* dm, const int32_t* order, const float* pupil,
+                          const float* amp, const uint8_t* valid, int B, int nS, int n, float phase_scale, float* frame,
+                          int32_t* envmax, double* stats, const SlopesTail& tail, void* stream);
+
+struct CommandUpdate {
+  const float* action;
+  const int32_t* act_idx;
+  float* coefs;
+  float* dm_prev;
+  float leak;
+  int nAct2;
+};
+int dm_rows_command(int ldc, const int32_t* act_pos, int nA, int nAct, int nActP, const float* wx, const int32_t* j0x, int W,
+                    int B, int R, float* rows, const CommandUpdate& cmd, void* stream);
+
+}
diff --git a/rlao_b200/csrc/ctrl.cu b/rlao_b200/csrc/ctrl.cu
--- a/rlao_b200/csrc/ctrl.cu
+++ b/rlao_b200/csrc/ctrl.cu
@@ -9,8 +9,7 @@
   const int b = blockIdx.y;
   const int a = blockIdx.x * blockDim.x + threadIdx.x;
   if (a >= nA) return;
-  const float act = __ldg(&action[(size_t)b * nAct2 + __ldg(&act_idx[a])]) * 1e-6f;
-  const float c = dm_prev[(size_t)b * ldc + a] * leak + act;
+  const float c = command_value(__ldg(&action[(size_t)b * nAct2 + __ldg(&act_idx[a])]), dm_prev[(size_t)b * ldc + a], leak);
   coefs[(size_t)b * ldc + a] = c;
   dm_prev[(size_t)b * ldc + a] = c;
 }
diff --git a/rlao_b200/csrc/step.cu b/rlao_b200/csrc/step.cu
--- a/rlao_b200/csrc/step.cu
+++ b/rlao_b200/csrc/step.cu
@@ -1,4 +1,5 @@
 #include <math.h>
+#include <stdlib.h>
 #include <string.h>
 
 #include "common.cuh"
@@ -172,6 +173,13 @@
 
 }
 
+static std::atomic<int> g_sh_fuse{[] {
+  const char* v = getenv("AOENV_SH_FUSE");
+  return (v != nullptr && v[0] == '0') ? 0 : 1;
+}()};
+
+extern "C" int aoenv_set_sh_fuse(int enabled) { return g_sh_fuse.exchange(enabled ? 1 : 0); }
+
 extern "C" int aoenv_sh_step(const aoenv_sh_step_t* c, int parts, const float* opd_a, const float* dm_rows_cur,
                              const aoenv_detector_t* det, const float* action, float* coefs_next, float* dm_rows_next,
                              float* obs, float* reward, float* strehl, float* total, float* residual, void* stream) {
@@ -180,6 +188,7 @@
   AOENV_CHECK_ARG(!(parts & 2) || (obs != nullptr && reward != nullptr && strehl != nullptr), "sh_step: null output argument");
   AOENV_CHECK_ARG(!(parts & 4) || (action != nullptr && coefs_next != nullptr && dm_rows_next != nullptr), "sh_step: null command argument");
   const bool tc = c->use_tc && c->B > AOENV_SKINNY_MAX_ROWS;
+  const bool fuse = g_sh_fuse.load(std::memory_order_relaxed) != 0;
   int rc = 0;
   if ((parts & 1) && c->geometric) {
     aoenv_dm_sep_t dm = c->dm;
@@ -188,6 +197,15 @@
                                c->nV, c->B, c->nS, c->n, c->phase_scale, c->inv_units, (float*)c->slopes, c->lds,
                                tc ? c->slope_planes : nullptr, 2, (double*)c->stats, stream);
     if (rc) return rc;
+  } else if ((parts & 1) && fuse && det == nullptr && c->arrivals != nullptr) {
+    aoenv_dm_sep_t dm = c->dm;
+    dm.rows = dm_rows_cur;
+    const SlopesTail tail{(int32_t*)c->arrivals, (const int32_t*)c->valid_idx, (const float*)c->ref_xy, (float*)c->slopes,
+                          tc ? (__nv_bfloat16*)c->slope_planes : nullptr, c->inv_units, c->threshold_cog, c->nV, c->lds, 2};
+    rc = shwfs_frame_dm_slopes(opd_a, &dm, (const int32_t*)c->order, (const float*)c->pupil, (const float*)c->amp,
+                               (const uint8_t*)c->valid, c->B, c->nS, c->n, c->phase_scale, (float*)c->frame,
+                               (int32_t*)c->envmax, (double*)c->stats, tail, stream);
+    if (rc) return rc;
   } else if (parts & 1) {
     aoenv_dm_sep_t dm = c->dm;
     dm.rows = dm_rows_cur;
@@ -212,7 +230,11 @@
                        c->n_pupil, c->phase_scale, obs, reward, strehl, total, residual, stream);
     if (rc) return rc;
   }
-  if (parts & 4) {
+  if ((parts & 4) && fuse) {
+    const CommandUpdate cmd{action, (const int32_t*)c->act_idx, coefs_next, (float*)c->dm_prev, c->leak, c->nAct2};
+    rc = dm_rows_command(c->ldc, (const int32_t*)c->act_pos, c->nA, c->nAct, c->dm.nActP, (const float*)c->wx,
+                         (const int32_t*)c->j0x, c->W, c->B, c->nS * c->n, dm_rows_next, cmd, stream);
+  } else if (parts & 4) {
     rc = aoenv_command_update(action, (const int32_t*)c->act_idx, c->B, c->nA, c->nAct2, c->leak, coefs_next, (float*)c->dm_prev,
                               c->ldc, stream);
     if (rc) return rc;
diff --git a/rlao_b200/csrc/wfs.cu b/rlao_b200/csrc/wfs.cu
--- a/rlao_b200/csrc/wfs.cu
+++ b/rlao_b200/csrc/wfs.cu
@@ -258,13 +258,65 @@
   }
 }
 
-template <int n, int WL = 0>
+template <int n>
+__device__ __forceinline__ void lenslet_slopes(const float2 (&v)[n][n / 2], float thr, int t, int b, int nV,
+                                               const float* __restrict__ ref_xy, float inv_units, float* __restrict__ slopes,
+                                               int lds, __nv_bfloat16* __restrict__ planes, size_t plane_stride, int parts) {
+  float s = 0.f, sx = 0.f, sy = 0.f;
+#pragma unroll
+  for (int p = 0; p < n; ++p)
+#pragma unroll
+    for (int q = 0; q < n; ++q) {
+      float x = (q & 1) ? v[p][q >> 1].y : v[p][q >> 1].x;
+      x = x < thr ? 0.f : x;
+      s += x;
+      sx = fmaf(x, (float)p, sx);
+      sy = fmaf(x, (float)q, sy);
+    }
+  float cx = sx / s, cy = sy / s;
+  if (!isfinite(cx)) cx = 0.f;
+  if (!isfinite(cy)) cy = 0.f;
+  const float sx_ = (cx - __ldg(&ref_xy[t])) * inv_units, sy_ = (cy - __ldg(&ref_xy[nV + t])) * inv_units;
+  slopes[(size_t)b * lds + t] = sx_;
+  slopes[(size_t)b * lds + nV + t] = sy_;
+  if (planes != nullptr) {
+    store_bf16_planes(planes, plane_stride, (size_t)b * lds + t, parts, sx_);
+    store_bf16_planes(planes, plane_stride, (size_t)b * lds + nV + t, parts, sy_);
+  }
+}
+
+template <int n>
+__device__ __forceinline__ void slopes_tail(const float* img, const int32_t* envmax, int nS, int b, const SlopesTail& tl) {
+  const int R = nS * n;
+  const float thr = tl.threshold_cog * ordered_to_float(__ldcg(&envmax[b]));
+  const size_t plane_stride = (size_t)gridDim.y * tl.lds;
+  for (int t0 = threadIdx.x; t0 < tl.nV; t0 += 2 * blockDim.x) {
+    const int t1 = t0 + blockDim.x;
+    const bool two = t1 < tl.nV;
+    float2 v[2][n][n / 2];
+#pragma unroll
+    for (int j = 0; j < 2; ++j) {
+      const int k = __ldg(&tl.valid_idx[(j == 1 && two) ? t1 : t0]);
+      const int li = k / nS, lj = k - li * nS;
+      const float* f = img + (size_t)(li * n) * R + lj * n;
+#pragma unroll
+      for (int p = 0; p < n; ++p)
+#pragma unroll
+        for (int h = 0; h < n / 2; ++h) v[j][p][h] = __ldcg(reinterpret_cast<const float2*>(f + (size_t)p * R) + h);
+    }
+    lenslet_slopes<n>(v[0], thr, t0, b, tl.nV, tl.ref_xy, tl.inv_units, tl.slopes, tl.lds, tl.planes, plane_stride, tl.parts);
+    if (two)
+      lenslet_slopes<n>(v[1], thr, t1, b, tl.nV, tl.ref_xy, tl.inv_units, tl.slopes, tl.lds, tl.planes, plane_stride, tl.parts);
+  }
+}
+
+template <int n, int WL = 0, bool kSlopes = false>
 __global__ void __launch_bounds__(128)
 shwfs_frame_kernel(const float* __restrict__ opd_a, const float* __restrict__ opd_b, const float* __restrict__ pupil,
                    const float* __restrict__ amp, const uint8_t* __restrict__ valid, int nS, float phase_scale,
                    int track_max, int shared_max, float* __restrict__ frame,
                    int32_t* __restrict__ envmax, double* __restrict__ stats, const __grid_constant__ aoenv_dm_sep_t dm,
-                   const int32_t* __restrict__ order) {
+                   const int32_t* __restrict__ order, const __grid_constant__ SlopesTail tail) {
   constexpr int N = 2 * n;
   pdl_enter();
   const int R = nS * n;
@@ -435,6 +487,18 @@
   if (track_max) {
     vmax = warp_max(vmax);
     if ((threadIdx.x & 31) == 0 && vmax > -INFINITY) atomicMax(&envmax[shared_max ? 0 : b], float_to_ordered(vmax));
+  }
+  if constexpr (kSlopes) {
+    __shared__ int last;
+    __syncthreads();
+    if (threadIdx.x == 0) {
+      int arrived;
+      asm volatile("atom.add.release.gpu.s32 %0, [%1], 1;" : "=r"(arrived) : "l"(&tail.arrivals[b]) : "memory");
+      if (arrived == (int)gridDim.x - 1) asm volatile("fence.acq_rel.gpu;" ::: "memory");
+      last = arrived == (int)gridDim.x - 1;
+    }
+    __syncthreads();
+    if (last) slopes_tail<n>(frame + (size_t)b * R * R, envmax, nS, b, tail);
   }
 }
 
@@ -914,27 +978,7 @@
   for (int p = 0; p < n; ++p)
 #pragma unroll
     for (int h = 0; h < n / 2; ++h) v[p][h] = __ldg(reinterpret_cast<const float2*>(f + (size_t)p * R) + h);
-  float s = 0.f, sx = 0.f, sy = 0.f;
-#pragma unroll
-  for (int p = 0; p < n; ++p)
-#pragma unroll
-    for (int q = 0; q < n; ++q) {
-      float x = (q & 1) ? v[p][q >> 1].y : v[p][q >> 1].x;
-      x = x < thr ? 0.f : x;
-      s += x;
-      sx = fmaf(x, (float)p, sx);
-      sy = fmaf(x, (float)q, sy);
-    }
-  float cx = sx / s, cy = sy / s;
-  if (!isfinite(cx)) cx = 0.f;
-  if (!isfinite(cy)) cy = 0.f;
-  const float sx_ = (cx - __ldg(&ref_xy[t])) * inv_units, sy_ = (cy - __ldg(&ref_xy[nV + t])) * inv_units;
-  slopes[(size_t)b * lds + t] = sx_;
-  slopes[(size_t)b * lds + nV + t] = sy_;
-  if (planes != nullptr) {
-    store_bf16_planes(planes, (size_t)gridDim.y * lds, (size_t)b * lds + t, parts, sx_);
-    store_bf16_planes(planes, (size_t)gridDim.y * lds, (size_t)b * lds + nV + t, parts, sy_);
-  }
+  lenslet_slopes<n>(v, thr, t, b, nV, ref_xy, inv_units, slopes, lds, planes, (size_t)gridDim.y * lds, parts);
 }
 
 template <int n>
@@ -1039,10 +1083,12 @@
   slopes[(size_t)b * lds + nV + t] = (cy - ref_xy[nV + t]) * inv_units;
 }
 
-__global__ void envmax_init_kernel(int32_t* __restrict__ envmax, int count, double* __restrict__ stats, int n_stats) {
+__global__ void envmax_init_kernel(int32_t* __restrict__ envmax, int count, double* __restrict__ stats, int n_stats,
+                                   int32_t* __restrict__ arrivals) {
   pdl_enter();
   const int i = blockIdx.x * blockDim.x + threadIdx.x;
   if (i < count) envmax[i] = float_to_ordered(-INFINITY);
+  if (arrivals != nullptr && i < count) arrivals[i] = 0;
   if (stats != nullptr && i < n_stats) stats[i] = 0.0;
 }
 
@@ -1059,17 +1105,33 @@
   return kDefaultFrameVariant;
 }()};
 
-extern "C" {
-
-int aoenv_set_wfs6_variant(int variant) {
-  return g_wfs6_factorised.exchange(variant < 0 || variant > 3 ? kDefaultFrameVariant : variant);
+template <int n, int WL>
+static void launch_frame_sep(dim3 grid, cudaStream_t s, const float* opd_a, const float* opd_b, const float* pupil,
+                             const float* amp, const uint8_t* valid, int nS, float phase_scale, int track_max, int shared_max,
+                             float* frame, int32_t* envmax, double* stats, const aoenv_dm_sep_t& dm, const int32_t* order,
+                             const SlopesTail* tail) {
+  if (tail != nullptr)
+    AOENV_LAUNCH((shwfs_frame_kernel<n, WL, true>), grid, 128, 0, s, opd_a, opd_b, pupil, amp, valid, nS, phase_scale, track_max,
+                 shared_max, frame, envmax, stats, dm, order, *tail);
+  else
+    AOENV_LAUNCH((shwfs_frame_kernel<n, WL>), grid, 128, 0, s, opd_a, opd_b, pupil, amp, valid, nS, phase_scale, track_max,
+                 shared_max, frame, envmax, stats, dm, order, SlopesTail{});
 }
 
 static int shwfs_frame_impl(const float* opd_a, const float* opd_b, const aoenv_dm_sep_t* dm_in, const int32_t* order, const float* pupil,
                             const float* amp, const uint8_t* valid, int B, int nS, int n, float phase_scale,
                             const aoenv_detector_t* det, int shared_max, float* frame, int32_t* envmax, double* stats,
-                            void* stream) {
+                            const SlopesTail* tail, void* stream) {
   AOENV_CHECK_ARG(B > 0 && B <= 65535 && nS > 0, "shwfs_frame: bad shape B=%d nS=%d", B, nS);
+  if (tail != nullptr) {
+    AOENV_CHECK_ARG(dm_in != nullptr && det == nullptr && shared_max == 0,
+                    "shwfs_frame_dm_slopes: needs the separable DM, the ideal detector and per-environment maxima");
+    AOENV_CHECK_ARG(tail->arrivals != nullptr && tail->valid_idx != nullptr && tail->ref_xy != nullptr && tail->slopes != nullptr &&
+                    tail->nV > 0 && tail->lds >= 2 * tail->nV, "shwfs_frame_dm_slopes: bad slopes arguments nV=%d lds=%d",
+                    tail->nV, tail->lds);
+    AOENV_CHECK_ARG(tail->planes == nullptr || tail->parts == 2 || tail->parts == 3, "shwfs_frame_dm_slopes: parts must be 2 or 3");
+    AOENV_CHECK_ARG((reinterpret_cast<uintptr_t>(frame) & 7) == 0, "shwfs_frame_dm_slopes: frame must be 8-byte aligned");
+  }
   aoenv_dm_sep_t dm{};
   if (dm_in != nullptr) {
     dm = *dm_in;
@@ -1087,7 +1149,8 @@
   }
   int rc = ensure_twiddles(n, s);
   if (rc) return rc;
-  AOENV_LAUNCH(envmax_init_kernel, dim3((4 * B + 255) / 256), 256, 0, s, envmax, shared_max ? 1 : B, stats, stats ? 4 * B : 0);
+  AOENV_LAUNCH(envmax_init_kernel, dim3((4 * B + 255) / 256), 256, 0, s, envmax, shared_max ? 1 : B, stats, stats ? 4 * B : 0,
+               tail ? tail->arrivals : nullptr);
   AOENV_LAUNCH_CHECK("envmax_init");
   dim3 grid((nS * nS + 127) / 128, B);
   const int variant = g_wfs6_factorised.load(std::memory_order_relaxed);
@@ -1101,26 +1164,26 @@
 #define AOENV_WFS_CASE(NN)                                                                                   \
   case NN:                                                                                                   \
     if (dm.WL == 14)                                                                                         \
-      AOENV_LAUNCH((shwfs_frame_kernel<NN, 14>), grid, 128, 0, s, opd_a, opd_b, pupil, amp, valid, nS, phase_scale, \
-                   (int)(det == nullptr), shared_max, frame, envmax, stats, dm, order);                             \
+      launch_frame_sep<NN, 14>(grid, s, opd_a, opd_b, pupil, amp, valid, nS, phase_scale, (int)(det == nullptr), shared_max, \
+                               frame, envmax, stats, dm, order, tail);                                      \
     else if (dm.WL == 18)                                                                                    \
-      AOENV_LAUNCH((shwfs_frame_kernel<NN, 18>), grid, 128, 0, s, opd_a, opd_b, pupil, amp, valid, nS, phase_scale, \
-                   (int)(det == nullptr), shared_max, frame, envmax, stats, dm, order);                             \
+      launch_frame_sep<NN, 18>(grid, s, opd_a, opd_b, pupil, amp, valid, nS, phase_scale, (int)(det == nullptr), shared_max, \
+                               frame, envmax, stats, dm, order, tail);                                      \
     else                                                                                                     \
       AOENV_LAUNCH((shwfs_frame_kernel<NN, 0>), grid, 128, 0, s, opd_a, opd_b, pupil, amp, valid, nS, phase_scale,  \
-                   (int)(det == nullptr), shared_max, frame, envmax, stats, dm, order);                             \
+                   (int)(det == nullptr), shared_max, frame, envmax, stats, dm, order, SlopesTail{});               \
     break;
   switch (n) {
     AOENV_WFS_CASE(4)
     AOENV_WFS_CASE(8)
     case 6:
       if (dm.WL != 0) {
-        if (dm.WL == 14) {
-          AOENV_LAUNCH((shwfs_frame_kernel<6, 14>), grid, 128, 0, s, opd_a, opd_b, pupil, amp, valid, nS, phase_scale,
-                       (int)(det == nullptr), shared_max, frame, envmax, stats, dm, order);
-        } else
-          AOENV_LAUNCH((shwfs_frame_kernel<6, 18>), grid, 128, 0, s, opd_a, opd_b, pupil, amp, valid, nS, phase_scale,
-                       (int)(det == nullptr), shared_max, frame, envmax, stats, dm, order);
+        if (dm.WL == 14)
+          launch_frame_sep<6, 14>(grid, s, opd_a, opd_b, pupil, amp, valid, nS, phase_scale, (int)(det == nullptr), shared_max,
+                                  frame, envmax, stats, dm, order, tail);
+        else
+          launch_frame_sep<6, 18>(grid, s, opd_a, opd_b, pupil, amp, valid, nS, phase_scale, (int)(det == nullptr), shared_max,
+                                  frame, envmax, stats, dm, order, tail);
       } else if (variant == 2) {
         dim3 g3((nS * nS + kS6Warps * kS6Lenslets - 1) / (kS6Warps * kS6Lenslets), B);
         shwfs_frame6s_kernel<<<g3, kS6Warps * 32, 0, s>>>(opd_a, opd_b, pupil, amp, valid, nS, phase_scale, det == nullptr,
@@ -1130,7 +1193,7 @@
                                                  frame, envmax, stats);
       else
         AOENV_LAUNCH((shwfs_frame_kernel<6, 0>), grid, 128, 0, s, opd_a, opd_b, pupil, amp, valid, nS, phase_scale,
-                     (int)(det == nullptr), shared_max, frame, envmax, stats, dm, order);
+                     (int)(det == nullptr), shared_max, frame, envmax, stats, dm, order, SlopesTail{});
       break;
   }
 #undef AOENV_WFS_CASE
@@ -1145,17 +1208,32 @@
   return 0;
 }
 
+int aoenv::shwfs_frame_dm_slopes(const float* opd_a, const aoenv_dm_sep_t* dm, const int32_t* order, const float* pupil,
+                                 const float* amp, const uint8_t* valid, int B, int nS, int n, float phase_scale, float* frame,
+                                 int32_t* envmax, double* stats, const SlopesTail& tail, void* stream) {
+  return shwfs_frame_impl(opd_a, nullptr, dm, order, pupil, amp, valid, B, nS, n, phase_scale, nullptr, 0, frame, envmax, stats,
+                          &tail, stream);
+}
+
+extern "C" {
+
+int aoenv_set_wfs6_variant(int variant) {
+  return g_wfs6_factorised.exchange(variant < 0 || variant > 3 ? kDefaultFrameVariant : variant);
+}
+
 int aoenv_shwfs_frame(const float* opd_a, const float* opd_b, const float* pupil, const float* amp,
                       const uint8_t* valid, int B, int nS, int n, float phase_scale, const aoenv_detector_t* det,
                       int shared_max, float* frame, int32_t* envmax, double* stats, void* stream) {
-  return shwfs_frame_impl(opd_a, opd_b, nullptr, nullptr, pupil, amp, valid, B, nS, n, phase_scale, det, shared_max, frame, envmax, stats, stream);
+  return shwfs_frame_impl(opd_a, opd_b, nullptr, nullptr, pupil, amp, valid, B, nS, n, phase_scale, det, shared_max, frame, envmax, stats,
+                          nullptr, stream);
 }
 
 int aoenv_shwfs_frame_dm(const float* opd_a, const float* opd_b, const aoenv_dm_sep_t* dm, const int32_t* order,
                          const float* pupil, const float* amp, const uint8_t* valid, int B, int nS, int n, float phase_scale,
                          const aoenv_detector_t* det, int shared_max, float* frame, int32_t* envmax, double* stats,
                          void* stream) {
-  return shwfs_frame_impl(opd_a, opd_b, dm, order, pupil, amp, valid, B, nS, n, phase_scale, det, shared_max, frame, envmax, stats, stream);
+  return shwfs_frame_impl(opd_a, opd_b, dm, order, pupil, amp, valid, B, nS, n, phase_scale, det, shared_max, frame, envmax, stats,
+                          nullptr, stream);
 }
 
 int aoenv_shwfs_camera(float* frame, const uint8_t* valid, int B, int nS, int n, const aoenv_detector_t* det, int shared_max,
@@ -1167,7 +1245,8 @@
   const int R = nS * n;
   AOENV_CHECK_ARG(R * R < (1 << 24), "shwfs_camera: frame of %d x %d pixels is too large for the camera pass", R, R);
   cudaStream_t s = (cudaStream_t)stream;
-  AOENV_LAUNCH(envmax_init_kernel, dim3((B + 255) / 256), 256, 0, s, envmax, shared_max ? 1 : B, (double*)nullptr, 0);
+  AOENV_LAUNCH(envmax_init_kernel, dim3((B + 255) / 256), 256, 0, s, envmax, shared_max ? 1 : B, (double*)nullptr, 0,
+               (int32_t*)nullptr);
   AOENV_LAUNCH_CHECK("envmax_init");
   dim3 gd((R * R + 8 * kDetPerLane * 32 - 1) / (8 * kDetPerLane * 32), B);
   shwfs_detector_kernel<<<gd, 256, 0, s>>>(frame, valid, nS, n, 1.0f / (float)R, 1.0f / (float)n, *det, shared_max, envmax, 0);
diff --git a/rlao_b200/csrc/wfs_fused.cu b/rlao_b200/csrc/wfs_fused.cu
--- a/rlao_b200/csrc/wfs_fused.cu
+++ b/rlao_b200/csrc/wfs_fused.cu
@@ -442,19 +442,48 @@
   if (p.frame != nullptr && tid == 64) asm volatile("cp.async.bulk.wait_group.read 0;" ::: "memory");
 }
 
-template <int W>
+template <int W, bool kCommand = false>
 __global__ void __launch_bounds__(256)
 dm_rows_kernel(const float* __restrict__ coefs, int ldc, const int32_t* __restrict__ act_pos, int nA, int nAct, int nActP,
-               const float* __restrict__ wx, const int32_t* __restrict__ j0x, int R, float* __restrict__ rows) {
+               const float* __restrict__ wx, const int32_t* __restrict__ j0x, int R, float* __restrict__ rows,
+               const __grid_constant__ CommandUpdate cmd) {
   pdl_enter();
   extern __shared__ __align__(16) float sC[];
   const int b = blockIdx.x, ldC = nAct + W;
   for (int k = threadIdx.x; k < nAct * ldC; k += blockDim.x) sC[k] = 0.f;
   __syncthreads();
-  for (int k = threadIdx.x; k < nA; k += blockDim.x) {
-    const int pos = __ldg(&act_pos[k]);
-    const int r = pos / nAct;
-    sC[r * ldC + (pos - r * nAct)] = __ldg(&coefs[(size_t)b * ldc + k]);
+  if constexpr (kCommand) {
+    constexpr int U = 4;
+    for (int k0 = threadIdx.x; k0 < nA; k0 += U * blockDim.x) {
+      float act[U], prev[U];
+      int pos[U];
+#pragma unroll
+      for (int u = 0; u < U; ++u) {
+        const int k = k0 + u * blockDim.x;
+        if (k < nA) {
+          pos[u] = __ldg(&act_pos[k]);
+          act[u] = __ldg(&cmd.action[(size_t)b * cmd.nAct2 + __ldg(&cmd.act_idx[k])]);
+          prev[u] = cmd.dm_prev[(size_t)b * ldc + k];
+        }
+      }
+#pragma unroll
+      for (int u = 0; u < U; ++u) {
+        const int k = k0 + u * blockDim.x;
+        if (k < nA) {
+          const float c = command_value(act[u], prev[u], cmd.leak);
+          cmd.coefs[(size_t)b * ldc + k] = c;
+          cmd.dm_prev[(size_t)b * ldc + k] = c;
+          const int r = pos[u] / nAct;
+          sC[r * ldC + (pos[u] - r * nAct)] = c;
+        }
+      }
+    }
+  } else {
+    for (int k = threadIdx.x; k < nA; k += blockDim.x) {
+      const int pos = __ldg(&act_pos[k]);
+      const int r = pos / nAct;
+      sC[r * ldC + (pos - r * nAct)] = __ldg(&coefs[(size_t)b * ldc + k]);
+    }
   }
   __syncthreads();
   float* __restrict__ out = rows + (size_t)b * nActP * R;
@@ -506,28 +535,40 @@
 
 using namespace aoenv;
 
-extern "C" {
-
-int aoenv_shwfs_fused_smem(int nS, int n, int rows_max, int groups, int t_rows, int WL) {
-  if (nS <= 0 || rows_max <= 0 || rows_max > nS || (n != 4 && n != 6 && n != 8)) return -1;
-  return fused_smem_layout(nS, n, rows_max, groups, t_rows, WL > 0 ? WL : 14, t_rows > 0).total;
-}
-
-int aoenv_dm_rows(const float* coefs, int ldc, const int32_t* act_pos, int nA, int nAct, int nActP, const float* wx,
-                  const int32_t* j0x, int W, int B, int R, float* rows, void* stream) {
+static int dm_rows_impl(const float* coefs, int ldc, const int32_t* act_pos, int nA, int nAct, int nActP, const float* wx,
+                        const int32_t* j0x, int W, int B, int R, float* rows, const CommandUpdate* cmd, void* stream) {
   AOENV_CHECK_ARG(B > 0 && R > 0 && nAct > 0 && nA > 0 && nA <= nAct * nAct && ldc >= nA && nActP >= nAct, "dm_rows: bad shape");
   AOENV_CHECK_ARG(W == 12 || W == 16, "dm_rows: band width %d (12 or 16)", W);
   const size_t smem = (size_t)nAct * (nAct + W) * sizeof(float);
   AOENV_CHECK_ARG(smem <= 200 * 1024, "dm_rows: %d actuators across do not fit in shared memory", nAct);
   cudaStream_t s = (cudaStream_t)stream;
-  cudaError_t e = W == 12 ? cudaFuncSetAttribute(dm_rows_kernel<12>, cudaFuncAttributeMaxDynamicSharedMemorySize, (int)smem)
-                          : cudaFuncSetAttribute(dm_rows_kernel<16>, cudaFuncAttributeMaxDynamicSharedMemorySize, (int)smem);
+  auto kern = W == 12 ? (cmd ? dm_rows_kernel<12, true> : dm_rows_kernel<12, false>)
+                      : (cmd ? dm_rows_kernel<16, true> : dm_rows_kernel<16, false>);
+  cudaError_t e = cudaFuncSetAttribute(kern, cudaFuncAttributeMaxDynamicSharedMemorySize, (int)smem);
   if (e != cudaSuccess) return fail(-3, "dm_rows smem attribute: %s", cudaGetErrorString(e));
   const dim3 grid(B, 1);
-  if (W == 12) AOENV_LAUNCH(dm_rows_kernel<12>, grid, 256, smem, s, coefs, ldc, act_pos, nA, nAct, nActP, wx, j0x, R, rows);
-  else AOENV_LAUNCH(dm_rows_kernel<16>, grid, 256, smem, s, coefs, ldc, act_pos, nA, nAct, nActP, wx, j0x, R, rows);
+  AOENV_LAUNCH(kern, grid, 256, smem, s, coefs, ldc, act_pos, nA, nAct, nActP, wx, j0x, R, rows, cmd ? *cmd : CommandUpdate{});
   AOENV_LAUNCH_CHECK("dm_rows");
   return 0;
+}
+
+int aoenv::dm_rows_command(int ldc, const int32_t* act_pos, int nA, int nAct, int nActP, const float* wx, const int32_t* j0x,
+                           int W, int B, int R, float* rows, const CommandUpdate& cmd, void* stream) {
+  AOENV_CHECK_ARG(cmd.action != nullptr && cmd.act_idx != nullptr && cmd.coefs != nullptr && cmd.dm_prev != nullptr &&
+                  cmd.nAct2 >= nA, "dm_rows_command: bad command arguments");
+  return dm_rows_impl(nullptr, ldc, act_pos, nA, nAct, nActP, wx, j0x, W, B, R, rows, &cmd, stream);
+}
+
+extern "C" {
+
+int aoenv_shwfs_fused_smem(int nS, int n, int rows_max, int groups, int t_rows, int WL) {
+  if (nS <= 0 || rows_max <= 0 || rows_max > nS || (n != 4 && n != 6 && n != 8)) return -1;
+  return fused_smem_layout(nS, n, rows_max, groups, t_rows, WL > 0 ? WL : 14, t_rows > 0).total;
+}
+
+int aoenv_dm_rows(const float* coefs, int ldc, const int32_t* act_pos, int nA, int nAct, int nActP, const float* wx,
+                  const int32_t* j0x, int W, int B, int R, float* rows, void* stream) {
+  return dm_rows_impl(coefs, ldc, act_pos, nA, nAct, nActP, wx, j0x, W, B, R, rows, nullptr, stream);
 }
 
 int aoenv_shwfs_fused(const float* opd_a, const float* opd_b, const aoenv_dm_sep_t* dm, const uint8_t* pupil8, float amp0,
```

Result: slower. 1.371 million, median of 6 (-2.7%).
